# ChainBreak/denoising_diffusion_deep_fake

Hardware: AMD Instinct MI355X
Metric: training images/sec (256x256 U-Net, bs=16/GPU) (higher is better)
Workload: dtype f32; 1 GPU; d3f train_denoiser step: noise blend -> Unet(resnet34) fwd -> (MSE+1-SSIM)/2 -> bwd -> Adam, 256x256 synthetic face crops, bs=16/GPU, random-init weights, train-mode BatchNorm; image_size=256, batch_per_gpu=16, global_batch=16, parallelism=dp1, graph_step=False, adam_overlap_tail=False, adam_overlap_tail_steps=0, ranks_seen=1, csrc_digest=830583e7fcebca8c

## Files before the change

### denoising_diffusion_deep_fake_amd/csrc/batchnorm.hip

```cpp
#include "common.h"
#include "pointwise.h"
#include "vec16.h"

#include <algorithm>
#include <type_traits>

namespace d3f {

constexpr float BN_EPS = 1e-5f, BN_MOMENTUM = 0.1f;

constexpr int BNF_SC = 32;
constexpr int BNF_MAX_ROWS = 1024;
#ifndef BNF_FWD_U_F32
#define BNF_FWD_U_F32 4
#endif
#ifndef BNF_BWD_U
#define BNF_BWD_U 2
#endif

__device__ __forceinline__ float2 bn_fwd_coef(double s1, double s2, double count, int c, const float* __restrict__ gamma,
                                              const float* __restrict__ beta, float eps, float momentum, bool store,
                                              float* __restrict__ running_mean, float* __restrict__ running_var,
                                              float* __restrict__ mean_o, float* __restrict__ invstd_o,
                                              float* __restrict__ scale_o, float* __restrict__ shift_o) {
  const double mean = s1 / count;
  double var = s2 / count - mean * mean;
  if (var < 0.0) var = 0.0;
  const double invstd = 1.0 / sqrt(var + (double)eps);
  const float g = gamma[c], bt = beta[c];
  const float sc = (float)((double)g * invstd), sf = (float)((double)bt - mean * (double)g * invstd);
  if (store) {
    mean_o[c] = (float)mean; invstd_o[c] = (float)invstd; scale_o[c] = sc; shift_o[c] = sf;
    if (running_mean != nullptr) {
      const double unbiased = count > 1.0 ? var * count / (count - 1.0) : var;
      running_mean[c] = (float)((1.0 - (double)momentum) * (double)running_mean[c] + (double)momentum * mean);
      running_var[c] = (float)((1.0 - (double)momentum) * (double)running_var[c] + (double)momentum * unbiased);
    }
  }
  return make_float2(sc, sf);
}

__device__ __forceinline__ float3 bn_bwd_coef(double s1, double s2, double count, int c, int C,
                                              const float* __restrict__ gamma, const float* __restrict__ invstd, bool store,
                                              float* __restrict__ dgamma, float* __restrict__ dbeta, float* __restrict__ k) {
  const float k0 = gamma[c] * invstd[c], k1 = (float)(s1 / count), k2 = (float)(s2 / count);
  if (store) {
    if (dgamma != nullptr) { dgamma[c] = (float)s2; dbeta[c] = (float)s1; }
    k[c] = k0; k[C + c] = k1; k[2 * C + c] = k2;
  }
  return make_float3(k0, k1, k2);
}

template <typename F> static void by_dtype(int dtype, F&& f) {
  if (dtype == D3F_F32) f((float*)nullptr);
  else f((bf16_t*)nullptr);
}

__device__ __forceinline__ void block_sum2(double& s1, double& s2) {
  __shared__ double red[2][4];
#pragma unroll
  for (int o = 32; o > 0; o >>= 1) {
    s1 += __shfl_xor(s1, o);
    s2 += __shfl_xor(s2, o);
  }
  if ((threadIdx.x & 63) == 0) {
    red[0][threadIdx.x >> 6] = s1;
    red[1][threadIdx.x >> 6] = s2;
  }
  __syncthreads();
  s1 = (red[0][0] + red[0][1]) + (red[0][2] + red[0][3]);
  s2 = (red[1][0] + red[1][1]) + (red[1][2] + red[1][3]);
}

__global__ __launch_bounds__(256) void bn_finalize_kernel(
    const float* __restrict__ stats, int tiles, int C, int Cpad, double count,
    const float* __restrict__ gamma, const float* __restrict__ beta, float eps, float momentum,
    float* __restrict__ running_mean, float* __restrict__ running_var, float* __restrict__ mean_o,
    float* __restrict__ invstd_o, float* __restrict__ scale_o, float* __restrict__ shift_o, NetSplit ns) {
  chain_priority();
  if (blockIdx.z != 0) {
    net_shift(stats, ns.ws); net_shift(gamma, ns.par); net_shift(beta, ns.par);
    net_shift(running_mean, ns.bn); net_shift(running_var, ns.bn);
    net_shift(mean_o, ns.ws); net_shift(invstd_o, ns.ws); net_shift(scale_o, ns.ws); net_shift(shift_o, ns.ws);
  }
  const int c = blockIdx.x;
  double s1 = 0.0, s2 = 0.0;
  for (int t = threadIdx.x; t < tiles; t += 256) {
    const float2 v = *reinterpret_cast<const float2*>(stats + ((long)t * Cpad + c) * 2);
    s1 += (double)v.x;
    s2 += (double)v.y;
  }
  block_sum2(s1, s2);
  if (threadIdx.x == 0)
    bn_fwd_coef(s1, s2, count, c, gamma, beta, eps, momentum, true, running_mean, running_var, mean_o, invstd_o, scale_o,
                shift_o);
}

__global__ __launch_bounds__(256) void bn_eval_coeff_all_kernel(const float* __restrict__ params,
                                                                const float* __restrict__ bnstats,
                                                                char* __restrict__ ws, float eps, BnEvalTable t) {
  const BnEvalEntry e = t.e[blockIdx.x];
  float* __restrict__ coef = reinterpret_cast<float*>(ws + (size_t)e.coef_off16 * 16);
  for (int c = threadIdx.x; c < e.C; c += 256) {
    const float invstd = 1.0f / sqrtf(bnstats[e.rv_off + c] + eps);
    const float sc = params[e.g_off + c] * invstd;
    coef[2 * e.C + c] = sc;
    coef[3 * e.C + c] = params[e.b_off + c] - bnstats[e.rm_off + c] * sc;
  }
}

static_assert(BN_SCALE == 2 && BN_SHIFT == 3, "bn_eval_coeff_all_kernel writes the scale / shift rows");
int bn_eval_coeff_all_launch(const float* params, const float* bnstats, void* ws, const BnEvalTable& t,
                             hipStream_t stream) {
  if (t.n == 0) return 0;
  hipLaunchKernelGGL(bn_eval_coeff_all_kernel, dim3(t.n), dim3(256), 0, stream, params, bnstats, (char*)ws, BN_EPS, t);
  D3F_HIP(hipGetLastError());
  return 0;
}

template <typename T>
__global__ __launch_bounds__(256) void bn_apply_kernel(
    const T* __restrict__ y, const float* __restrict__ scale, const float* __restrict__ shift,
    const T* __restrict__ res, const T* __restrict__ yr, const float* __restrict__ scale_r,
    const float* __restrict__ shift_r, int relu, T* __restrict__ out, long nvec, int C, long net_ws) {
  chain_priority();
  if (blockIdx.z != 0) {
    net_shift(y, net_ws); net_shift(scale, net_ws); net_shift(shift, net_ws); net_shift(res, net_ws); net_shift(yr, net_ws);
    net_shift(scale_r, net_ws); net_shift(shift_r, net_ws); net_shift(out, net_ws);
  }
  constexpr int N = V16<T>::N;
  for (long i = (long)blockIdx.x * 256 + threadIdx.x; i < nvec; i += (long)gridDim.x * 256) {
    const int c0 = (int)((i * N) % C);
    float v[N], sc[N], sf[N];
    V16<T>::load(y + i * N, v);
#pragma unroll
    for (int k = 0; k < N; k += 4) {
      const float4 a = *reinterpret_cast<const float4*>(scale + c0 + k);
      const float4 b = *reinterpret_cast<const float4*>(shift + c0 + k);
      sc[k] = a.x; sc[k + 1] = a.y; sc[k + 2] = a.z; sc[k + 3] = a.w;
      sf[k] = b.x; sf[k + 1] = b.y; sf[k + 2] = b.z; sf[k + 3] = b.w;
    }
#pragma unroll
    for (int k = 0; k < N; ++k) v[k] = v[k] * sc[k] + sf[k];
    if (res != nullptr) {
      float r[N];
      V16<T>::load(res + i * N, r);
#pragma unroll
      for (int k = 0; k < N; ++k) v[k] += r[k];
    } else if (yr != nullptr) {
      float r[N];
      V16<T>::load(yr + i * N, r);
#pragma unroll
      for (int k = 0; k < N; ++k) v[k] += r[k] * scale_r[c0 + k] + shift_r[c0 + k];
    }
    if (relu) {
#pragma unroll
      for (int k = 0; k < N; ++k) v[k] = fmaxf(v[k], 0.f);
    }
    V16<T>::store(out + i * N, v);
  }
}



template <typename T>
__global__ __launch_bounds__(256) void bn_bwd_reduce_kernel(
    const T* __restrict__ dA, const T* __restrict__ a, const T* __restrict__ y,
    const float* __restrict__ mean, const float* __restrict__ invstd, float* __restrict__ partial,
    long rows, int C, const float* __restrict__ mask_scale, const float* __restrict__ mask_shift, long net_ws) {
  chain_priority();
  if (blockIdx.z != 0) {
    net_shift(dA, net_ws); net_shift(a, net_ws); net_shift(y, net_ws); net_shift(mean, net_ws); net_shift(invstd, net_ws);
    net_shift(partial, net_ws); net_shift(mask_scale, net_ws); net_shift(mask_shift, net_ws);
  }
  constexpr int N = V16<T>::N;
  __shared__ float red[256 * N * 2];
  const int VC = C / N;
  const int RP = 256 / VC;
  const int cv = threadIdx.x % VC, r0 = threadIdx.x / VC;
  const long rows_per_block = (rows + gridDim.x - 1) / gridDim.x;
  const long rbeg = (long)blockIdx.x * rows_per_block;
  long rend = rbeg + rows_per_block;
  if (rend > rows) rend = rows;
  float mu[N], is[N], s1[N], s2[N], msc[N], msf[N];
#pragma unroll
  for (int k = 0; k < N; ++k) {
    mu[k] = mean[cv * N + k];
    is[k] = invstd[cv * N + k];
    msc[k] = mask_scale ? mask_scale[cv * N + k] : 0.f;
    msf[k] = mask_scale ? mask_shift[cv * N + k] : 0.f;
    s1[k] = 0.f;
    s2[k] = 0.f;
  }
  constexpr int U = 4;
  const bool from_y = mask_scale != nullptr, from_a = !from_y && a != nullptr;
  long r = rbeg + r0;
  for (; r + (U - 1) * RP < rend; r += U * RP) {
    float g[U][N], yy[U][N], aa[U][N];
#pragma unroll
    for (int u = 0; u < U; ++u) {
      const long off = (r + u * RP) * C + cv * N;
      V16<T>::load(dA + off, g[u]);
      V16<T>::load(y + off, yy[u]);
      if (from_a) V16<T>::load(a + off, aa[u]);
    }
#pragma unroll
    for (int u = 0; u < U; ++u) {
#pragma unroll
      for (int k = 0; k < N; ++k) {
        const float keep = from_y ? yy[u][k] * msc[k] + msf[k] : (from_a ? aa[u][k] : 1.f);
        const float gz = keep > 0.f ? g[u][k] : 0.f;
        s1[k] += gz;
        s2[k] += gz * ((yy[u][k] - mu[k]) * is[k]);
      }
    }
  }
  for (; r < rend; r += RP) {
    const long off = r * C + cv * N;
    float g[N], yy[N], aa[N];
    V16<T>::load(dA + off, g);
    V16<T>::load(y + off, yy);
    if (from_a) V16<T>::load(a + off, aa);
#pragma unroll
    for (int k = 0; k < N; ++k) {
      const float keep = from_y ? yy[k] * msc[k] + msf[k] : (from_a ? aa[k] : 1.f);
      const float gz = keep > 0.f ? g[k] : 0.f;
      s1[k] += gz;
      s2[k] += gz * ((yy[k] - mu[k]) * is[k]);
    }
  }
#pragma unroll
  for (int k = 0; k < N; ++k) {
    red[(threadIdx.x * N + k) * 2 + 0] = s1[k];
    red[(threadIdx.x * N + k) * 2 + 1] = s2[k];
  }
  __syncthreads();
  for (int t = threadIdx.x; t < 2 * C; t += 256) {
    const int c = t >> 1, which = t & 1;
    const int v = c / N, k = c % N;
    float s = 0.f;
    for (int rr = 0; rr < RP; ++rr) s += red[((rr * VC + v) * N + k) * 2 + which];
    partial[((long)blockIdx.x * C + c) * 2 + which] = s;
  }
}

__global__ __launch_bounds__(256) void bn_bwd_finalize_kernel(
    const float* __restrict__ partial, int nblocks, int C, double count,
    const float* __restrict__ gamma, const float* __restrict__ invstd, float* __restrict__ dgamma,
    float* __restrict__ dbeta, float* __restrict__ coef, NetSplit ns) {
  chain_priority();
  if (blockIdx.z != 0) {
    net_shift(partial, ns.ws); net_shift(gamma, ns.par); net_shift(invstd, ns.ws);
    net_shift(dgamma, ns.grad); net_shift(dbeta, ns.grad); net_shift(coef, ns.ws);
  }
  const int c = blockIdx.x;
  double s1 = 0.0, s2 = 0.0;
  for (int t = threadIdx.x; t < nblocks; t += 256) {
    const float2 v = *reinterpret_cast<const float2*>(partial + ((long)t * C + c) * 2);
    s1 += (double)v.x;
    s2 += (double)v.y;
  }
  block_sum2(s1, s2);
  if (threadIdx.x == 0) bn_bwd_coef(s1, s2, count, c, C, gamma, invstd, true, dgamma, dbeta, coef);
}

template <typename T>
__global__ __launch_bounds__(256) void bn_bwd_apply_kernel(
    const T* __restrict__ dA, const T* __restrict__ a, const T* __restrict__ y,
    const float* __restrict__ mean, const float* __restrict__ invstd, const float* __restrict__ coef,
    T* __restrict__ dy, T* __restrict__ dres, int dres_acc, long nvec, int C,
    const float* __restrict__ mask_scale, const float* __restrict__ mask_shift, long net_ws) {
  chain_priority();
  if (blockIdx.z != 0) {
    net_shift(dA, net_ws); net_shift(a, net_ws); net_shift(y, net_ws); net_shift(mean, net_ws); net_shift(invstd, net_ws);
    net_shift(coef, net_ws); net_shift(dy, net_ws); net_shift(dres, net_ws); net_shift(mask_scale, net_ws);
    net_shift(mask_shift, net_ws);
  }
  constexpr int N = V16<T>::N;
  for (long i = (long)blockIdx.x * 256 + threadIdx.x; i < nvec; i += (long)gridDim.x * 256) {
    const int c0 = (int)((i * N) % C);
    float g[N], yy[N], o[N];
    V16<T>::load(dA + i * N, g);
    V16<T>::load(y + i * N, yy);
    if (mask_scale != nullptr) {
#pragma unroll
      for (int k = 0; k < N; ++k) g[k] = (yy[k] * mask_scale[c0 + k] + mask_shift[c0 + k]) > 0.f ? g[k] : 0.f;
    } else if (a != nullptr) {
      float aa[N];
      V16<T>::load(a + i * N, aa);
#pragma unroll
      for (int k = 0; k < N; ++k) g[k] = aa[k] > 0.f ? g[k] : 0.f;
    }
#pragma unroll
    for (int k = 0; k < N; ++k) {
      const int c = c0 + k;
      const float xhat = (yy[k] - mean[c]) * invstd[c];
      o[k] = coef[c] * (g[k] - coef[C + c] - xhat * coef[2 * C + c]);
    }
    V16<T>::store(dy + i * N, o);
    if (dres != nullptr) {
      if (dres_acc) {
        float d[N];
        V16<T>::load(dres + i * N, d);
#pragma unroll
        for (int k = 0; k < N; ++k) g[k] += d[k];
      }
      V16<T>::store(dres + i * N, g);
    }
  }
}

template <typename T> struct Raw4;
template <> struct Raw4<float> { typedef float4 type; };
template <> struct Raw4<bf16_t> { typedef uint2 type; };
__device__ __forceinline__ float4 ldraw(const float* p) { return *reinterpret_cast<const float4*>(p); }
__device__ __forceinline__ uint2 ldraw(const bf16_t* p) { return *reinterpret_cast<const uint2*>(p); }
__device__ __forceinline__ float4 cvt4(const float4& v) { return v; }
__device__ __forceinline__ float4 cvt4(const uint2& v) {
  return make_float4(__uint_as_float(v.x << 16), __uint_as_float(v.x & 0xffff0000u), __uint_as_float(v.y << 16),
                     __uint_as_float(v.y & 0xffff0000u));
}

template <typename F>
__device__ __forceinline__ void slab_reduce(const float* __restrict__ partial, int rows, int ld, int c0,
                                            double (&red)[16][64], double (&tot)[64], F behind_first_loads) {
  const int tid = threadIdx.x, q = tid & 15, rl = tid >> 4;
  double a0 = 0.0, a1 = 0.0, a2 = 0.0, a3 = 0.0;
  const float* base = partial + ((long)c0 * 2 + q * 4);
  int r = rl;
  bool hooked = false;
  for (; r + 112 < rows; r += 128) {
    float4 v[8];
#pragma unroll
    for (int j = 0; j < 8; ++j) v[j] = *reinterpret_cast<const float4*>(base + (long)(r + 16 * j) * ld * 2);
    if (!hooked) { behind_first_loads(); hooked = true; }
#pragma unroll
    for (int j = 0; j < 8; ++j) {
      a0 += (double)v[j].x; a1 += (double)v[j].y; a2 += (double)v[j].z; a3 += (double)v[j].w;
    }
  }
  for (; r + 48 < rows; r += 64) {
    const float4 v0 = *reinterpret_cast<const float4*>(base + (long)r * ld * 2);
    const float4 v1 = *reinterpret_cast<const float4*>(base + (long)(r + 16) * ld * 2);
    const float4 v2 = *reinterpret_cast<const float4*>(base + (long)(r + 32) * ld * 2);
    const float4 v3 = *reinterpret_cast<const float4*>(base + (long)(r + 48) * ld * 2);
    if (!hooked) { behind_first_loads(); hooked = true; }
    a0 += (double)v0.x; a1 += (double)v0.y; a2 += (double)v0.z; a3 += (double)v0.w;
    a0 += (double)v1.x; a1 += (double)v1.y; a2 += (double)v1.z; a3 += (double)v1.w;
    a0 += (double)v2.x; a1 += (double)v2.y; a2 += (double)v2.z; a3 += (double)v2.w;
    a0 += (double)v3.x; a1 += (double)v3.y; a2 += (double)v3.z; a3 += (double)v3.w;
  }
  if (!hooked) behind_first_loads();
  for (; r < rows; r += 16) {
    const float4 v = *reinterpret_cast<const float4*>(base + (long)r * ld * 2);
    a0 += (double)v.x; a1 += (double)v.y; a2 += (double)v.z; a3 += (double)v.w;
  }
  red[rl][q * 4 + 0] = a0;
  red[rl][q * 4 + 1] = a1;
  red[rl][q * 4 + 2] = a2;
  red[rl][q * 4 + 3] = a3;
  __syncthreads();
  if (tid < 64) {
    double s = 0.0;
#pragma unroll
    for (int k = 0; k < 16; ++k) s += red[k][tid];
    tot[tid] = s;
  }
  __syncthreads();
}

template <typename T, bool HAS2>
__global__ __launch_bounds__(256) void bn_finalize_apply_kernel(
    const float* __restrict__ stats, int stat_rows, int C, int Cpad, double count,
    const float* __restrict__ gamma, const float* __restrict__ beta, float eps, float momentum,
    float* __restrict__ running_mean, float* __restrict__ running_var, float* __restrict__ mean_o,
    float* __restrict__ invstd_o, float* __restrict__ scale_o, float* __restrict__ shift_o,
    const T* __restrict__ y, const T* __restrict__ res, const T* __restrict__ yr,
    const float* __restrict__ scale_r, const float* __restrict__ shift_r, int relu, T* __restrict__ out,
    long rows, long rows_per_block, NetSplit ns) {
  chain_priority();
  if (blockIdx.z != 0) {
    net_shift(stats, ns.ws); net_shift(gamma, ns.par); net_shift(beta, ns.par);
    net_shift(running_mean, ns.bn); net_shift(running_var, ns.bn);
    net_shift(mean_o, ns.ws); net_shift(invstd_o, ns.ws); net_shift(scale_o, ns.ws); net_shift(shift_o, ns.ws);
    net_shift(y, ns.ws); net_shift(res, ns.ws); net_shift(yr, ns.ws); net_shift(scale_r, ns.ws); net_shift(shift_r, ns.ws);
    net_shift(out, ns.ws);
  }
  __shared__ double red[16][64];
  __shared__ double tot[64];
  __shared__ float cf[2][BNF_SC];
  typedef typename Raw4<T>::type raw_t;
  constexpr int U = sizeof(T) == 4 ? BNF_FWD_U_F32 : 8;
  const int tid = threadIdx.x, c0 = blockIdx.y * BNF_SC;
  const int v = tid & 7, rr = tid >> 3, cc = c0 + v * 4;
  const long r0 = (long)blockIdx.x * rows_per_block;
  long r1 = r0 + rows_per_block;
  if (r1 > rows) r1 = rows;
  const T* __restrict__ second = res != nullptr ? res : yr;
  raw_t a[U], b[U], an[U], bn[U];
  auto load = [&](raw_t (&ya)[U], raw_t (&yb)[U], long r) {
#pragma unroll
    for (int u = 0; u < U; ++u) {
      const long row = r + 32 * u < r1 ? r + 32 * u : r1 - 1;
      ya[u] = ldraw(y + row * C + cc);
      if (HAS2) yb[u] = ldraw(second + row * C + cc);
    }
  };
  slab_reduce(stats, stat_rows, Cpad, c0, red, tot, [&]() { load(a, b, r0 + rr); });
  if (tid < BNF_SC) {
    const float2 f = bn_fwd_coef(tot[2 * tid], tot[2 * tid + 1], count, c0 + tid, gamma, beta, eps, momentum,
                                 blockIdx.x == 0, running_mean, running_var, mean_o, invstd_o, scale_o, shift_o);
    cf[0][tid] = f.x;
    cf[1][tid] = f.y;
  }
  __syncthreads();
  float sc[4], sf[4], scr[4] = {0.f, 0.f, 0.f, 0.f}, sfr[4] = {0.f, 0.f, 0.f, 0.f};
#pragma unroll
  for (int k = 0; k < 4; ++k) {
    sc[k] = cf[0][v * 4 + k];
    sf[k] = cf[1][v * 4 + k];
    if (HAS2 && res == nullptr) {
      scr[k] = scale_r[cc + k];
      sfr[k] = shift_r[cc + k];
    }
  }
  for (long r = r0 + rr; r < r1; r += 32 * U) {
    if (r + 32 * U < r1) load(an, bn, r + 32 * U);
#pragma unroll
    for (int u = 0; u < U; ++u) {
      const long row = r + 32 * u;
      if (row >= r1) continue;
      const float4 ya = cvt4(a[u]);
      float x[4] = {ya.x, ya.y, ya.z, ya.w};
#pragma unroll
      for (int k = 0; k < 4; ++k) x[k] = x[k] * sc[k] + sf[k];
      if (HAS2) {
        const float4 yb = cvt4(b[u]);
        if (res != nullptr) {
          x[0] += yb.x; x[1] += yb.y; x[2] += yb.z; x[3] += yb.w;
        } else {
          const float t[4] = {yb.x, yb.y, yb.z, yb.w};
#pragma unroll
          for (int k = 0; k < 4; ++k) x[k] += t[k] * scr[k] + sfr[k];
        }
      }
      if (relu) {
#pragma unroll
        for (int k = 0; k < 4; ++k) x[k] = fmaxf(x[k], 0.f);
      }
      st4<T>(out + row * C + cc, make_float4(x[0], x[1], x[2], x[3]));
    }
#pragma unroll
    for (int u = 0; u < U; ++u) {
      a[u] = an[u];
      if (HAS2) b[u] = bn[u];
    }
  }
}

static long rows_per_block_for(long rows, int slabs, int dtype, int plan_nets) {
  const long wgs = (dtype == D3F_F32 ? 256 : 512) / plan_nets_for(plan_nets, 64);
  long rb = std::max(1L, wgs / slabs);
  long rpb = (rows + rb - 1) / rb;
  rpb = (rpb + 31) / 32 * 32;
  return std::max(32L, rpb);
}

struct BnResidualOps {
  const void *res = nullptr, *yr = nullptr;
  const float *scale_r = nullptr, *shift_r = nullptr;
};
static BnResidualOps residual_ops(const BnLayer& L, const BnBufs& b) {
  if (L.res == BN_RES_TENSOR) return {b.res, nullptr, nullptr, nullptr};
  if (L.res == BN_RES_LAYER) return {nullptr, b.res, bn_coef(b.res_coef, L.C, BN_SCALE), bn_coef(b.res_coef, L.C, BN_SHIFT)};
  return {};
}

static int bn_finalize_apply_launch(const BnLayer& L, const BnBufs& b, hipStream_t stream, const NetSplit* ns) {
  if (L.rows == 0) return 0;
  const NetSplit nv = net_split_or_single(ns);
  const dim3 grid((unsigned)((L.rows + L.rows_per_block - 1) / L.rows_per_block), (unsigned)(L.C / BNF_SC),
                  (unsigned)nv.nets);
  const BnResidualOps r = residual_ops(L, b);
  by_dtype(L.dtype, [&](auto* typed) {
    typedef std::remove_pointer_t<decltype(typed)> T;
    auto go = [&](auto kernel) {
      hipLaunchKernelGGL(kernel, grid, dim3(256), 0, stream, b.stats, L.fwd_rows, L.C, L.Cpad, (double)L.rows, b.gamma,
                         b.beta, BN_EPS, BN_MOMENTUM, b.running_mean, b.running_var, bn_coef(b.coef, L.C, BN_MEAN),
                         bn_coef(b.coef, L.C, BN_INVSTD), bn_coef(b.coef, L.C, BN_SCALE), bn_coef(b.coef, L.C, BN_SHIFT),
                         (const T*)b.y, (const T*)r.res, (const T*)r.yr, r.scale_r, r.shift_r, L.relu ? 1 : 0, (T*)b.a,
                         L.rows, L.rows_per_block, nv);
    };
    if (L.res != BN_RES_NONE) go(bn_finalize_apply_kernel<T, true>);
    else go(bn_finalize_apply_kernel<T, false>);
  });
  D3F_HIP(hipGetLastError());
  return 0;
}

template <typename T, bool FROM_A, bool RD_DRES>
__global__ __launch_bounds__(256) void bn_bwd_finalize_apply_kernel(
    const float* __restrict__ partial, int nblocks, int C, double count, const float* __restrict__ gamma,
    const float* __restrict__ mean, const float* __restrict__ invstd, float* __restrict__ dgamma,
    float* __restrict__ dbeta, float* __restrict__ coef, const T* __restrict__ dA,
    const T* __restrict__ a, const T* __restrict__ y, T* __restrict__ dy, T* __restrict__ dres,
    long rows, long rows_per_block, const float* __restrict__ mask_scale,
    const float* __restrict__ mask_shift, NetSplit ns) {
  chain_priority();
  if (blockIdx.z != 0) {
    net_shift(partial, ns.ws); net_shift(gamma, ns.par); net_shift(mean, ns.ws); net_shift(invstd, ns.ws);
    net_shift(dgamma, ns.grad); net_shift(dbeta, ns.grad); net_shift(coef, ns.ws);
    net_shift(dA, ns.ws); net_shift(a, ns.ws); net_shift(y, ns.ws); net_shift(dy, ns.ws); net_shift(dres, ns.ws);
    net_shift(mask_scale, ns.ws); net_shift(mask_shift, ns.ws);
  }
  __shared__ double red[16][64];
  __shared__ double tot[64];
  __shared__ float cf[3][BNF_SC];
  typedef typename Raw4<T>::type raw_t;
  constexpr int U = BNF_BWD_U;
  const int tid = threadIdx.x, c0 = blockIdx.y * BNF_SC;
  const int v = tid & 7, rr = tid >> 3, cc = c0 + v * 4;
  const long r0 = (long)blockIdx.x * rows_per_block;
  long r1 = r0 + rows_per_block;
  if (r1 > rows) r1 = rows;
  raw_t g4[U], y4[U], a4[U], d4[U], g4n[U], y4n[U], a4n[U], d4n[U];
  auto load = [&](raw_t (&gg)[U], raw_t (&yy)[U], raw_t (&aa)[U], raw_t (&dd)[U], long r) {
#pragma unroll
    for (int u = 0; u < U; ++u) {
      const long row = r + 32 * u < r1 ? r + 32 * u : r1 - 1;
      gg[u] = ldraw(dA + row * C + cc);
      yy[u] = ldraw(y + row * C + cc);
      if (FROM_A) aa[u] = ldraw(a + row * C + cc);
      if (RD_DRES) dd[u] = ldraw(dres + row * C + cc);
    }
  };
  slab_reduce(partial, nblocks, C, c0, red, tot, [&]() { load(g4, y4, a4, d4, r0 + rr); });
  if (tid < BNF_SC) {
    const float3 k = bn_bwd_coef(tot[2 * tid], tot[2 * tid + 1], count, c0 + tid, C, gamma, invstd, blockIdx.x == 0,
                                 dgamma, dbeta, coef);
    cf[0][tid] = k.x;
    cf[1][tid] = k.y;
    cf[2][tid] = k.z;
  }
  __syncthreads();
  float k0[4], k1[4], k2[4], mu[4], is[4], msc[4] = {0.f, 0.f, 0.f, 0.f}, msf[4] = {0.f, 0.f, 0.f, 0.f};
#pragma unroll
  for (int k = 0; k < 4; ++k) {
    k0[k] = cf[0][v * 4 + k];
    k1[k] = cf[1][v * 4 + k];
    k2[k] = cf[2][v * 4 + k];
    mu[k] = mean[cc + k];
    is[k] = invstd[cc + k];
    if (!FROM_A && mask_scale != nullptr) {
      msc[k] = mask_scale[cc + k];
      msf[k] = mask_shift[cc + k];
    }
  }
  for (long r = r0 + rr; r < r1; r += 32 * U) {
    if (r + 32 * U < r1) load(g4n, y4n, a4n, d4n, r + 32 * U);
#pragma unroll
    for (int u = 0; u < U; ++u) {
      const long row = r + 32 * u;
      if (row >= r1) continue;
      const float4 gv = cvt4(g4[u]), yv = cvt4(y4[u]);
      float g[4] = {gv.x, gv.y, gv.z, gv.w};
      const float yy[4] = {yv.x, yv.y, yv.z, yv.w};
      if (FROM_A) {
        const float4 av = cvt4(a4[u]);
        const float aa[4] = {av.x, av.y, av.z, av.w};
#pragma unroll
        for (int k = 0; k < 4; ++k) g[k] = aa[k] > 0.f ? g[k] : 0.f;
      } else if (mask_scale != nullptr) {
#pragma unroll
        for (int k = 0; k < 4; ++k) g[k] = (yy[k] * msc[k] + msf[k]) > 0.f ? g[k] : 0.f;
      }
      float o[4];
#pragma unroll
      for (int k = 0; k < 4; ++k) {
        const float xhat = (yy[k] - mu[k]) * is[k];
        o[k] = k0[k] * (g[k] - k1[k] - xhat * k2[k]);
      }
      st4<T>(dy + row * C + cc, make_float4(o[0], o[1], o[2], o[3]));
      if (dres != nullptr) {
        if (RD_DRES) {
          const float4 dv = cvt4(d4[u]);
          g[0] += dv.x; g[1] += dv.y; g[2] += dv.z; g[3] += dv.w;
        }
        st4<T>(dres + row * C + cc, make_float4(g[0], g[1], g[2], g[3]));
      }
    }
#pragma unroll
    for (int u = 0; u < U; ++u) {
      g4[u] = g4n[u];
      y4[u] = y4n[u];
      if (FROM_A) a4[u] = a4n[u];
      if (RD_DRES) d4[u] = d4n[u];
    }
  }
}

struct BnBwdOps {
  const float *mean, *invstd;
  float* k;
  const void* a;
  const float *mask_scale, *mask_shift;
};
static BnBwdOps bwd_ops(const BnLayer& L, const BnBufs& b) {
  const bool from_y = L.mask == BN_MASK_FROM_Y;
  return {bn_coef(b.coef, L.C, BN_MEAN), bn_coef(b.coef, L.C, BN_INVSTD), b.k != nullptr ? b.k : bn_coef(b.coef, L.C, BN_K),
          L.mask == BN_MASK_FROM_A ? b.a : nullptr, from_y ? bn_coef(b.coef, L.C, BN_SCALE) : nullptr,
          from_y ? bn_coef(b.coef, L.C, BN_SHIFT) : nullptr};
}

static int bn_bwd_finalize_apply_launch(const BnLayer& L, const BnBufs& b, const BnBwdOps& o, hipStream_t stream,
                                        const NetSplit* ns) {
  if (L.rows == 0) return 0;
  const NetSplit nv = net_split_or_single(ns);
  const dim3 grid((unsigned)((L.rows + L.rows_per_block - 1) / L.rows_per_block), (unsigned)(L.C / BNF_SC),
                  (unsigned)nv.nets);
  const bool from_a = o.mask_scale == nullptr && o.a != nullptr;
  const bool rd_dres = b.dres != nullptr && b.dres_acc;
  by_dtype(L.dtype, [&](auto* typed) {
    typedef std::remove_pointer_t<decltype(typed)> T;
    auto go = [&](auto kernel) {
      hipLaunchKernelGGL(kernel, grid, dim3(256), 0, stream, b.stats, L.bwd_rows, L.C, (double)L.rows, b.gamma, o.mean,
                         o.invstd, b.dgamma, b.dbeta, o.k, (const T*)b.dA, (const T*)o.a, (const T*)b.y, (T*)b.dy,
                         (T*)b.dres, L.rows, L.rows_per_block, o.mask_scale, o.mask_shift, nv);
    };
    if (from_a && rd_dres) go(bn_bwd_finalize_apply_kernel<T, true, true>);
    else if (from_a) go(bn_bwd_finalize_apply_kernel<T, true, false>);
    else if (rd_dres) go(bn_bwd_finalize_apply_kernel<T, false, true>);
    else go(bn_bwd_finalize_apply_kernel<T, false, false>);
  });
  D3F_HIP(hipGetLastError());
  return 0;
}

void bn_layer_plan(BnLayer& L) {
  static const bool no_fused = getenv("D3F_NO_BN_FUSED_FINALIZE") != nullptr;
  auto fused_ok = [&](int rows) {
    return L.allow_fused && !no_fused && (L.dtype == D3F_F32 || L.dtype == D3F_BF16) && L.C % BNF_SC == 0 && rows >= 1 &&
           rows <= BNF_MAX_ROWS;
  };
  const long min_rows = std::max(16L, 4L * (256 / std::max(1, std::min(256, L.C / (L.dtype == D3F_F32 ? 4 : 8)))));
  L.reduce_blocks = (int)std::clamp((L.rows + min_rows - 1) / min_rows, 1L, 1024L);
  L.bwd_rows = L.fused_rows > 0 ? L.fused_rows : L.reduce_blocks;
  L.fwd_fused = L.apply && fused_ok(L.fwd_rows);
  L.bwd_fused = fused_ok(L.bwd_rows);
  L.rows_per_block = L.fwd_fused || L.bwd_fused ? rows_per_block_for(L.rows, L.C / BNF_SC, L.dtype, L.plan_nets) : 0;
  L.stat_floats = (size_t)L.fwd_rows * L.Cpad * 2;
  L.part_floats = (size_t)std::max(L.reduce_blocks, L.fused_rows) * L.C * 2;
}

int bn_layer_finalize(const BnLayer& L, const BnBufs& b, long count, hipStream_t stream, const NetSplit* ns) {
  const NetSplit nv = net_split_or_single(ns);
  hipLaunchKernelGGL(bn_finalize_kernel, dim3(L.C, 1, nv.nets), dim3(256), 0, stream, b.stats, L.fwd_rows, L.C, L.Cpad,
                     (double)count, b.gamma, b.beta, BN_EPS, BN_MOMENTUM, b.running_mean, b.running_var,
                     bn_coef(b.coef, L.C, BN_MEAN), bn_coef(b.coef, L.C, BN_INVSTD), bn_coef(b.coef, L.C, BN_SCALE),
                     bn_coef(b.coef, L.C, BN_SHIFT), nv);
  D3F_HIP(hipGetLastError());
  return 0;
}

int bn_layer_apply(const BnLayer& L, const BnBufs& b, hipStream_t stream, const NetSplit* ns) {
  const int ve = L.dtype == D3F_F32 ? 4 : 8;
  D3F_CHECK(L.C % ve == 0 && (256 * ve) % L.C == 0, "bn_apply: C=%d must divide %d", L.C, 256 * ve);
  const long nvec = L.rows * L.C / ve;
  if (nvec == 0) return 0;
  const NetSplit nv = net_split_or_single(ns);
  const BnResidualOps r = residual_ops(L, b);
  by_dtype(L.dtype, [&](auto* typed) {
    typedef std::remove_pointer_t<decltype(typed)> T;
    hipLaunchKernelGGL(bn_apply_kernel<T>, dim3(grid_for(nvec), 1, nv.nets), dim3(256), 0, stream, (const T*)b.y,
                       bn_coef(b.coef, L.C, BN_SCALE), bn_coef(b.coef, L.C, BN_SHIFT), (const T*)r.res, (const T*)r.yr,
                       r.scale_r, r.shift_r, L.relu ? 1 : 0, (T*)b.a, nvec, L.C, nv.ws);
  });
  D3F_HIP(hipGetLastError());
  return 0;
}

int bn_layer_forward(const BnLayer& L, const BnBufs& b, const BnSync* sync, hipStream_t stream, const NetSplit* ns) {
  long count = L.rows;
  if (sync != nullptr) {
    if (int rc = sync->fn(sync->ctx, b.stats, (int64_t)L.fwd_rows * L.Cpad * 2, (void*)stream))
      return set_error(rc, "BatchNorm statistics all-reduce failed in the forward pass (%s)", L.name.c_str());
    count *= sync->world;
  } else if (L.fwd_fused) {
    return bn_finalize_apply_launch(L, b, stream, ns);
  }
  if (int rc = bn_layer_finalize(L, b, count, stream, ns)) return rc;
  return L.apply ? bn_layer_apply(L, b, stream, ns) : 0;
}

int bn_layer_backward(const BnLayer& L, const BnBufs& b, const BnSync* sync, hipStream_t stream, const NetSplit* ns) {
  const int C = L.C, ve = L.dtype == D3F_F32 ? 4 : 8, vc = C / ve;
  const NetSplit nv = net_split_or_single(ns);
  const BnBwdOps o = bwd_ops(L, b);
  if (L.fused_rows == 0) {
    D3F_CHECK(C % ve == 0 && vc >= 1 && vc <= 256 && (256 % vc) == 0, "bn_bwd_reduce: unsupported channel count %d", C);
    by_dtype(L.dtype, [&](auto* typed) {
      typedef std::remove_pointer_t<decltype(typed)> T;
      hipLaunchKernelGGL(bn_bwd_reduce_kernel<T>, dim3(L.reduce_blocks, 1, nv.nets), dim3(256), 0, stream,
                         (const T*)b.dA, (const T*)o.a, (const T*)b.y, o.mean, o.invstd, b.stats, L.rows, C, o.mask_scale,
                         o.mask_shift, nv.ws);
    });
    D3F_HIP(hipGetLastError());
  }
  auto finalize = [&](long count, float* dgamma, float* dbeta) -> int {
    hipLaunchKernelGGL(bn_bwd_finalize_kernel, dim3(C, 1, nv.nets), dim3(256), 0, stream, b.stats, L.bwd_rows, C,
                       (double)count, b.gamma, o.invstd, dgamma, dbeta, o.k, nv);
    D3F_HIP(hipGetLastError());
    return 0;
  };
  if (sync != nullptr) {
    if (int rc = finalize(L.rows, b.dgamma, b.dbeta)) return rc;
    if (int rc = sync->fn(sync->ctx, b.stats, (int64_t)L.bwd_rows * C * 2, (void*)stream))
      return set_error(rc, "BatchNorm statistics all-reduce failed in the backward pass (%s)", L.name.c_str());
    if (int rc = finalize(L.rows * sync->world, nullptr, nullptr)) return rc;
  } else if (L.bwd_fused) {
    return bn_bwd_finalize_apply_launch(L, b, o, stream, ns);
  } else if (int rc = finalize(L.rows, b.dgamma, b.dbeta)) {
    return rc;
  }
  D3F_CHECK(C % ve == 0 && (256 * ve) % C == 0, "bn_bwd_apply: C=%d must divide %d", C, 256 * ve);
  const long nvec = L.rows * C / ve;
  if (nvec == 0) return 0;
  by_dtype(L.dtype, [&](auto* typed) {
    typedef std::remove_pointer_t<decltype(typed)> T;
    hipLaunchKernelGGL(bn_bwd_apply_kernel<T>, dim3(grid_for(nvec), 1, nv.nets), dim3(256), 0, stream, (const T*)b.dA,
                       (const T*)o.a, (const T*)b.y, o.mean, o.invstd, o.k, (T*)b.dy, (T*)b.dres, b.dres_acc, nvec, C,
                       o.mask_scale, o.mask_shift, nv.ws);
  });
  D3F_HIP(hipGetLastError());
  return 0;
}

}
```

### denoising_diffusion_deep_fake_amd/csrc/loss.hip

```cpp
#include "pointwise.h"
#include "philox.h"

namespace d3f {

constexpr int SS_T = 32;
constexpr int SS_K = 11;
constexpr int SS_IN = SS_T + SS_K - 1;
constexpr int SS_LD = SS_IN + 1;

struct GaussK {
  float g[SS_K];
};

static GaussK make_gauss() {
  GaussK k;
  float s = 0.f;
  for (int i = 0; i < SS_K; ++i) {
    const float d = (float)i - (float)(SS_K - 1) / 2.f;
    k.g[i] = expf(-(d * d) / (2.f * 1.5f * 1.5f));
    s += k.g[i];
  }
  for (int i = 0; i < SS_K; ++i) k.g[i] /= s;
  return k;
}

__device__ __forceinline__ float norm01(float v, float lo, float range) {
  const float t = (v - lo) / range;
  return fminf(fmaxf(t, 0.f), 1.f);
}

__global__ __launch_bounds__(256) void ssim_fwd_kernel(const float* __restrict__ pred,
                                                       const float* __restrict__ target, float lo,
                                                       float range, GaussK gk, int H, int W,
                                                       float* __restrict__ dA, float* __restrict__ dB,
                                                       float* __restrict__ dC,
                                                       float* __restrict__ partial) {
  chain_priority();
  __shared__ float tx[SS_IN * SS_LD], ty[SS_IN * SS_LD];
  __shared__ float vv[5][SS_T * SS_LD];
  __shared__ float wsum[4];
  const int Hv = H - (SS_K - 1), Wv = W - (SS_K - 1);
  const int plane = blockIdx.z;
  const int oy0 = blockIdx.y * SS_T, ox0 = blockIdx.x * SS_T;
  const float* __restrict__ px = pred + (long)plane * H * W;
  const float* __restrict__ py = target + (long)plane * H * W;
  const int tid = threadIdx.x;
  for (int e = tid; e < SS_IN * SS_IN; e += 256) {
    const int r = e / SS_IN, c = e - r * SS_IN;
    const int iy = oy0 + r, ix = ox0 + c;
    float a = 0.f, b = 0.f;
    if (iy < H && ix < W) {
      a = norm01(px[(long)iy * W + ix], lo, range);
      b = norm01(py[(long)iy * W + ix], lo, range);
    }
    tx[r * SS_LD + c] = a;
    ty[r * SS_LD + c] = b;
  }
  __syncthreads();
  constexpr int RB = 8;
  if (tid < SS_IN * (SS_T / RB)) {
    const int c = tid % SS_IN, r0 = (tid / SS_IN) * RB;
    float a[RB + SS_K - 1], b[RB + SS_K - 1], aa[RB + SS_K - 1], bb[RB + SS_K - 1], ab[RB + SS_K - 1];
#pragma unroll
    for (int i = 0; i < RB + SS_K - 1; ++i) {
      a[i] = tx[(r0 + i) * SS_LD + c];
      b[i] = ty[(r0 + i) * SS_LD + c];
      aa[i] = a[i] * a[i];
      bb[i] = b[i] * b[i];
      ab[i] = a[i] * b[i];
    }
#pragma unroll
    for (int r = 0; r < RB; ++r) {
      float s0 = 0.f, s1 = 0.f, s2 = 0.f, s3 = 0.f, s4 = 0.f;
#pragma unroll
      for (int i = 0; i < SS_K; ++i) {
        const float g = gk.g[i];
        s0 += g * a[r + i];
        s1 += g * b[r + i];
        s2 += g * aa[r + i];
        s3 += g * bb[r + i];
        s4 += g * ab[r + i];
      }
      vv[0][(r0 + r) * SS_LD + c] = s0;
      vv[1][(r0 + r) * SS_LD + c] = s1;
      vv[2][(r0 + r) * SS_LD + c] = s2;
      vv[3][(r0 + r) * SS_LD + c] = s3;
      vv[4][(r0 + r) * SS_LD + c] = s4;
    }
  }
  __syncthreads();
  const float c1 = 0.01f * 0.01f, c2 = 0.03f * 0.03f;
  float local = 0.f;
  constexpr int CBk = 4;
  const int rr = tid / (SS_T / CBk), cq = (tid % (SS_T / CBk)) * CBk;
  float win[5][CBk + SS_K - 1];
#pragma unroll
  for (int q = 0; q < 5; ++q)
#pragma unroll
    for (int j = 0; j < CBk + SS_K - 1; ++j) win[q][j] = vv[q][rr * SS_LD + cq + j];
#pragma unroll
  for (int cc = 0; cc < CBk; ++cc) {
    const int r = rr, c = cq + cc;
    const int oy = oy0 + r, ox = ox0 + c;
    if (oy >= Hv || ox >= Wv) continue;
    float m[5];
#pragma unroll
    for (int q = 0; q < 5; ++q) {
      float s = 0.f;
#pragma unroll
      for (int j = 0; j < SS_K; ++j) s += gk.g[j] * win[q][cc + j];
      m[q] = s;
    }
    const float mux = m[0], muy = m[1];
    const float sxx = m[2] - mux * mux, syy = m[3] - muy * muy, sxy = m[4] - mux * muy;
    const float a1 = 2.f * mux * muy + c1, b1 = mux * mux + muy * muy + c1;
    const float a2 = 2.f * sxy + c2, b2 = sxx + syy + c2;
    const float l = a1 / b1, cs = a2 / b2;
    const float ss = l * cs;
    local += ss;
    const long o = ((long)plane * Hv + oy) * Wv + ox;
    const float dl_dmux = 2.f * (muy - l * mux) / b1;
    const float dcs_dmux = (2.f * mux * cs - 2.f * muy) / b2;
    dA[o] = cs * dl_dmux + l * dcs_dmux;
    dB[o] = -l * cs / b2;
    dC[o] = 2.f * l / b2;
  }
#pragma unroll
  for (int o = 32; o > 0; o >>= 1) local += __shfl_xor(local, o);
  if ((tid & 63) == 0) wsum[tid >> 6] = local;
  __syncthreads();
  if (tid == 0)
    partial[((long)blockIdx.z * gridDim.y + blockIdx.y) * gridDim.x + blockIdx.x] =
        (wsum[0] + wsum[1]) + (wsum[2] + wsum[3]);
}

__global__ __launch_bounds__(256) void ssim_mse_bwd_kernel(
    const float* __restrict__ pred, const float* __restrict__ target, float lo, float range, GaussK gk,
    int H, int W, const float* __restrict__ dA, const float* __restrict__ dB,
    const float* __restrict__ dC, float ssim_coef, float mse_coef, float* __restrict__ grad,
    float* __restrict__ partial_mse) {
  chain_priority();
  __shared__ float t3[3][SS_IN * SS_LD];
  __shared__ float vv[3][SS_T * SS_LD];
  __shared__ float wsum[4];
  const int Hv = H - (SS_K - 1), Wv = W - (SS_K - 1);
  const int plane = blockIdx.z;
  const int py0 = blockIdx.y * SS_T, px0 = blockIdx.x * SS_T;
  const int tid = threadIdx.x;
  for (int e = tid; e < SS_IN * SS_IN; e += 256) {
    const int r = e / SS_IN, c = e - r * SS_IN;
    const int oy = py0 - (SS_K - 1) + r, ox = px0 - (SS_K - 1) + c;
    float a = 0.f, b = 0.f, d = 0.f;
    if (oy >= 0 && oy < Hv && ox >= 0 && ox < Wv) {
      const long o = ((long)plane * Hv + oy) * Wv + ox;
      a = dA[o];
      b = dB[o];
      d = dC[o];
    }
    t3[0][r * SS_LD + c] = a;
    t3[1][r * SS_LD + c] = b;
    t3[2][r * SS_LD + c] = d;
  }
  __syncthreads();
  constexpr int RB = 8;
  if (tid < SS_IN * (SS_T / RB)) {
    const int c = tid % SS_IN, r0 = (tid / SS_IN) * RB;
    float v0[RB + SS_K - 1], v1[RB + SS_K - 1], v2[RB + SS_K - 1];
#pragma unroll
    for (int i = 0; i < RB + SS_K - 1; ++i) {
      v0[i] = t3[0][(r0 + i) * SS_LD + c];
      v1[i] = t3[1][(r0 + i) * SS_LD + c];
      v2[i] = t3[2][(r0 + i) * SS_LD + c];
    }
#pragma unroll
    for (int r = 0; r < RB; ++r) {
      float s0 = 0.f, s1 = 0.f, s2 = 0.f;
#pragma unroll
      for (int i = 0; i < SS_K; ++i) {
        const float g = gk.g[SS_K - 1 - i];
        s0 += g * v0[r + i];
        s1 += g * v1[r + i];
        s2 += g * v2[r + i];
      }
      vv[0][(r0 + r) * SS_LD + c] = s0;
      vv[1][(r0 + r) * SS_LD + c] = s1;
      vv[2][(r0 + r) * SS_LD + c] = s2;
    }
  }
  __syncthreads();
  const float inv_range = 1.f / range;
  float local = 0.f;
  constexpr int CBk = 4;
  const int rr = tid / (SS_T / CBk), cq = (tid % (SS_T / CBk)) * CBk;
  float win[3][CBk + SS_K - 1];
#pragma unroll
  for (int q = 0; q < 3; ++q)
#pragma unroll
    for (int j = 0; j < CBk + SS_K - 1; ++j) win[q][j] = vv[q][rr * SS_LD + cq + j];
#pragma unroll
  for (int cc = 0; cc < CBk; ++cc) {
    const int r = rr, c = cq + cc;
    const int iy = py0 + r, ix = px0 + c;
    if (iy >= H || ix >= W) continue;
    float ga = 0.f, gb = 0.f, gc = 0.f;
#pragma unroll
    for (int j = 0; j < SS_K; ++j) {
      const float g = gk.g[SS_K - 1 - j];
      ga += g * win[0][cc + j];
      gb += g * win[1][cc + j];
      gc += g * win[2][cc + j];
    }
    const long p = (long)plane * H * W + (long)iy * W + ix;
    const float pv = pred[p], tv = target[p];
    const float rawx = (pv - lo) / range;
    const float xh = fminf(fmaxf(rawx, 0.f), 1.f);
    const float yh = norm01(tv, lo, range);
    float gx = ga + 2.f * xh * gb + yh * gc;
    gx = (rawx >= 0.f && rawx <= 1.f) ? gx * inv_range : 0.f;
    const float diff = pv - tv;
    local += diff * diff;
    grad[p] = ssim_coef * gx + mse_coef * diff;
  }
#pragma unroll
  for (int o = 32; o > 0; o >>= 1) local += __shfl_xor(local, o);
  if ((tid & 63) == 0) wsum[tid >> 6] = local;
  __syncthreads();
  if (tid == 0)
    partial_mse[((long)blockIdx.z * gridDim.y + blockIdx.y) * gridDim.x + blockIdx.x] =
        (wsum[0] + wsum[1]) + (wsum[2] + wsum[3]);
}

__global__ __launch_bounds__(256) void loss_finalize_kernel(const float* __restrict__ part_ss, int n_ss,
                                                            const float* __restrict__ part_mse,
                                                            int n_mse, double n_ssim_elems,
                                                            double n_elems, float* __restrict__ out) {
  chain_priority();
  __shared__ double red[2][256];
  double a = 0.0, b = 0.0;
  for (int i = threadIdx.x; i < n_ss; i += 256) a += (double)part_ss[i];
  for (int i = threadIdx.x; i < n_mse; i += 256) b += (double)part_mse[i];
  red[0][threadIdx.x] = a;
  red[1][threadIdx.x] = b;
  __syncthreads();
  for (int s = 128; s > 0; s >>= 1) {
    if (threadIdx.x < s) {
      red[0][threadIdx.x] += red[0][threadIdx.x + s];
      red[1][threadIdx.x] += red[1][threadIdx.x + s];
    }
    __syncthreads();
  }
  if (threadIdx.x == 0) {
    const float ssim = (float)(red[0][0] / n_ssim_elems);
    const float mse = (float)(red[1][0] / n_elems);
    out[0] = (mse + (1.0f - ssim)) / 2.0f;
    out[1] = mse;
    out[2] = ssim;
  }
}

static inline int tiles(int n) { return (n + SS_T - 1) / SS_T; }

size_t loss_workspace_floats(int B, int H, int W) {
  if (H < SS_K || W < SS_K) return 0;
  const long planes = (long)B * 3;
  const long maps = 3 * planes * (H - SS_K + 1) * (W - SS_K + 1);
  const long p1 = planes * tiles(H - SS_K + 1) * tiles(W - SS_K + 1);
  const long p2 = planes * tiles(H) * tiles(W);
  return (size_t)(maps + p1 + p2 + 16);
}

int mse_ssim_loss_launch(const float* pred, const float* target, float in_min, float in_max,
                         float* loss_out, float* grad_pred, float* workspace, int B, int H, int W,
                         hipStream_t stream) {
  D3F_CHECK(H >= SS_K && W >= SS_K, "loss: image %dx%d smaller than the 11x11 SSIM window", H, W);
  D3F_CHECK(in_max > in_min, "loss: input range");
  static const GaussK gk = make_gauss();
  const int Hv = H - SS_K + 1, Wv = W - SS_K + 1;
  const long planes = (long)B * 3;
  const long map = planes * Hv * Wv;
  float* dA = workspace;
  float* dB = dA + map;
  float* dC = dB + map;
  float* part_ss = dC + map;
  const int n_ss = (int)(planes * tiles(Hv) * tiles(Wv));
  float* part_mse = part_ss + n_ss;
  const int n_mse = (int)(planes * tiles(H) * tiles(W));
  const float range = in_max - in_min;
  hipLaunchKernelGGL(ssim_fwd_kernel, dim3(tiles(Wv), tiles(Hv), (unsigned)planes), dim3(256), 0, stream,
                     pred, target, in_min, range, gk, H, W, dA, dB, dC, part_ss);
  D3F_HIP(hipGetLastError());
  const double n_elems = (double)planes * H * W;
  const double n_ssim = (double)planes * Hv * Wv;
  const float ssim_coef = (float)(-0.5 / n_ssim);
  const float mse_coef = (float)(1.0 / n_elems);
  hipLaunchKernelGGL(ssim_mse_bwd_kernel, dim3(tiles(W), tiles(H), (unsigned)planes), dim3(256), 0,
                     stream, pred, target, in_min, range, gk, H, W, dA, dB, dC, ssim_coef, mse_coef,
                     grad_pred, part_mse);
  D3F_HIP(hipGetLastError());
  hipLaunchKernelGGL(loss_finalize_kernel, dim3(1), dim3(256), 0, stream, part_ss, n_ss, part_mse, n_mse,
                     n_ssim, n_elems, loss_out);
  D3F_HIP(hipGetLastError());
  return 0;
}

struct BlendCoef {
  float r, sa, sb;
};
__device__ __forceinline__ BlendCoef blend_coef(float y, float c, float one_minus_c, float inv_lam) {
  const float t = __fadd_rn(__fmul_rn(y, one_minus_c), c);
  const float r = inv_lam > 0.f ? __fmul_rn(inv_lam, (float)log((double)__fdiv_rn(1.0f, t))) : y;
  return BlendCoef{r, __fsqrt_rn(__fsub_rn(1.0f, r)), __fsqrt_rn(r)};
}
__device__ __forceinline__ float4 blend4(const BlendCoef k, const float4 a, const float4 n) {
  float4 o;
  o.x = __fadd_rn(__fmul_rn(k.sa, a.x), __fmul_rn(k.sb, n.x));
  o.y = __fadd_rn(__fmul_rn(k.sa, a.y), __fmul_rn(k.sb, n.y));
  o.z = __fadd_rn(__fmul_rn(k.sa, a.z), __fmul_rn(k.sb, n.z));
  o.w = __fadd_rn(__fmul_rn(k.sa, a.w), __fmul_rn(k.sb, n.w));
  return o;
}

__global__ __launch_bounds__(256) void noise_blend_kernel(const float* __restrict__ x,
                                                          const float* __restrict__ noise,
                                                          const float* __restrict__ y_uniform,
                                                          float c, float one_minus_c, float inv_lam,
                                                          float* __restrict__ out,
                                                          float* __restrict__ r_out, long per_image) {
  const int b = blockIdx.y;
  const BlendCoef k = blend_coef(y_uniform[b], c, one_minus_c, inv_lam);
  if (r_out != nullptr && blockIdx.x == 0 && threadIdx.x == 0) r_out[b] = k.r;
  const long nvec = per_image / 4;
  const float4* __restrict__ xv = reinterpret_cast<const float4*>(x + (long)b * per_image);
  const float4* __restrict__ nv = reinterpret_cast<const float4*>(noise + (long)b * per_image);
  float4* __restrict__ ov = reinterpret_cast<float4*>(out + (long)b * per_image);
  for (long i = (long)blockIdx.x * 256 + threadIdx.x; i < nvec; i += (long)gridDim.x * 256) ov[i] = blend4(k, xv[i], nv[i]);
}

int noise_blend_launch(const float* x, const float* noise, const float* y_uniform, float lam,
                       float* out, float* r_out, int B, long per_image, hipStream_t stream) {
  D3F_CHECK(per_image % 4 == 0, "noise_blend: per-image element count %ld not a multiple of 4", per_image);
  D3F_CHECK(lam > 0.f, "noise_blend: lambda must be positive");
  if (B == 0 || per_image == 0) return 0;
  const double c = 1.0 / exp((double)lam);
  long bx = (per_image / 4 + 255) / 256;
  if (bx > 256) bx = 256;
  hipLaunchKernelGGL(noise_blend_kernel, dim3((unsigned)bx, (unsigned)B), dim3(256), 0, stream, x, noise,
                     y_uniform, (float)c, (float)(1.0 - c), (float)(1.0 / (double)lam), out, r_out,
                     per_image);
  D3F_HIP(hipGetLastError());
  return 0;
}

int noise_blend_fixed_launch(const float* x, const float* noise, const float* r, float* out, int B, long per_image,
                             hipStream_t stream) {
  D3F_CHECK(per_image % 4 == 0, "noise_blend: per-image element count %ld not a multiple of 4", per_image);
  if (B == 0 || per_image == 0) return 0;
  long bx = (per_image / 4 + 255) / 256;
  if (bx > 256) bx = 256;
  hipLaunchKernelGGL(noise_blend_kernel, dim3((unsigned)bx, (unsigned)B), dim3(256), 0, stream, x, noise, r, 0.f, 0.f,
                     -1.f, out, (float*)nullptr, per_image);
  D3F_HIP(hipGetLastError());
  return 0;
}

__global__ __launch_bounds__(256) void noise_blend_rng_kernel(const float* __restrict__ x, uint64_t seed, uint64_t offset,
                                                              const float* __restrict__ y_or_r, float c,
                                                              float one_minus_c, float inv_lam, float* __restrict__ out,
                                                              float* __restrict__ r_out, long per_image) {
  chain_priority();
  const int b = blockIdx.y;
  const BlendCoef k = blend_coef(y_or_r != nullptr ? y_or_r[b] : rng_y(seed, offset, b), c, one_minus_c, inv_lam);
  if (r_out != nullptr && blockIdx.x == 0 && threadIdx.x == 0) r_out[b] = k.r;
  const long nvec = per_image / 4;
  const float4* __restrict__ xv = reinterpret_cast<const float4*>(x + (long)b * per_image);
  float4* __restrict__ ov = reinterpret_cast<float4*>(out + (long)b * per_image);
  for (long i = (long)blockIdx.x * 256 + threadIdx.x; i < nvec; i += (long)gridDim.x * 256)
    ov[i] = blend4(k, xv[i], rng_normal4(seed, offset, b, (uint32_t)i));
}

__global__ __launch_bounds__(256) void noise_draw_kernel(uint64_t seed, uint64_t offset, float* __restrict__ noise,
                                                         float* __restrict__ y, long per_image) {
  const int b = blockIdx.y;
  if (y != nullptr && blockIdx.x == 0 && threadIdx.x == 0) y[b] = rng_y(seed, offset, b);
  if (noise == nullptr) return;
  const long nvec = per_image / 4;
  float4* __restrict__ nv = reinterpret_cast<float4*>(noise + (long)b * per_image);
  for (long i = (long)blockIdx.x * 256 + threadIdx.x; i < nvec; i += (long)gridDim.x * 256)
    nv[i] = rng_normal4(seed, offset, b, (uint32_t)i);
}

static int rng_shape_check(const char* what, long per_image) {
  D3F_CHECK(per_image % 4 == 0, "%s: per-image element count %ld not a multiple of 4", what, per_image);
  D3F_CHECK(per_image / 4 < (long)RNG_G_APPLY, "%s: per-image element count %ld leaves no room for the reserved groups",
            what, per_image);
  return 0;
}
static unsigned rng_blocks(long per_image) {
  const long bx = (per_image / 4 + 255) / 256;
  return (unsigned)(bx > 256 ? 256 : (bx < 1 ? 1 : bx));
}

int noise_blend_rng_launch(const float* x, uint64_t seed, uint64_t offset, float lam, float* out, float* r_out, int B,
                           long per_image, hipStream_t stream) {
  if (int rc = rng_shape_check("noise_blend_rng", per_image)) return rc;
  D3F_CHECK(lam > 0.f, "noise_blend_rng: lambda must be positive");
  if (B == 0 || per_image == 0) return 0;
  const double c = 1.0 / exp((double)lam);
  hipLaunchKernelGGL(noise_blend_rng_kernel, dim3(rng_blocks(per_image), (unsigned)B), dim3(256), 0, stream, x, seed,
                     offset, (const float*)nullptr, (float)c, (float)(1.0 - c), (float)(1.0 / (double)lam), out, r_out,
                     per_image);
  D3F_HIP(hipGetLastError());
  return 0;
}

int noise_blend_fixed_rng_launch(const float* x, uint64_t seed, uint64_t offset, const float* r, float* out, int B,
                                 long per_image, hipStream_t stream) {
  if (int rc = rng_shape_check("noise_blend_fixed_rng", per_image)) return rc;
  if (B == 0 || per_image == 0) return 0;
  hipLaunchKernelGGL(noise_blend_rng_kernel, dim3(rng_blocks(per_image), (unsigned)B), dim3(256), 0, stream, x, seed,
                     offset, r, 0.f, 0.f, -1.f, out, (float*)nullptr, per_image);
  D3F_HIP(hipGetLastError());
  return 0;
}

int noise_draw_launch(uint64_t seed, uint64_t offset, float* noise, float* y, int B, long per_image,
                      hipStream_t stream) {
  if (int rc = rng_shape_check("noise_draw", per_image)) return rc;
  if (B == 0 || (noise == nullptr && y == nullptr)) return 0;
  const unsigned bx = (noise != nullptr && per_image > 0) ? rng_blocks(per_image) : 1u;
  hipLaunchKernelGGL(noise_draw_kernel, dim3(bx, (unsigned)B), dim3(256), 0, stream, seed, offset,
                     per_image > 0 ? noise : (float*)nullptr, y, per_image);
  D3F_HIP(hipGetLastError());
  return 0;
}

__global__ __launch_bounds__(256) void l1_partial_kernel(const float* __restrict__ p, const float* __restrict__ t,
                                                         double* __restrict__ partial, long per_image) {
  __shared__ double red[256];
  const int b = blockIdx.y;
  const float* pp = p + (long)b * per_image;
  const float* tt = t + (long)b * per_image;
  double s = 0.0;
  for (long i = (long)blockIdx.x * 256 + threadIdx.x; i < per_image; i += (long)gridDim.x * 256)
    s += (double)fabsf(pp[i] - tt[i]);
  red[threadIdx.x] = s;
  __syncthreads();
  for (int o = 128; o > 0; o >>= 1) {
    if ((int)threadIdx.x < o) red[threadIdx.x] += red[threadIdx.x + o];
    __syncthreads();
  }
  if (threadIdx.x == 0) partial[(long)b * L1_PARTS + blockIdx.x] = red[0];
}
__global__ void l1_finalize_kernel(const double* __restrict__ partial, float* __restrict__ out, int B, long per_image) {
  const int b = blockIdx.x * blockDim.x + threadIdx.x;
  if (b >= B) return;
  out[b] = l1_image_mean(partial, b, per_image);
}
size_t l1_per_image_workspace_bytes(int B) { return (size_t)B * L1_PARTS * sizeof(double) + 64; }
int l1_partials_launch(const float* pred, const float* target, double* partial, int B, long per_image,
                       hipStream_t stream) {
  hipLaunchKernelGGL(l1_partial_kernel, dim3(L1_PARTS, (unsigned)B), dim3(256), 0, stream, pred, target, partial,
                     per_image);
  D3F_HIP(hipGetLastError());
  return 0;
}
int l1_per_image_launch(const float* pred, const float* target, float* out, void* workspace, int B, long per_image,
                        hipStream_t stream) {
  if (B == 0) return 0;
  double* partial = reinterpret_cast<double*>(workspace);
  if (int rc = l1_partials_launch(pred, target, partial, B, per_image, stream)) return rc;
  hipLaunchKernelGGL(l1_finalize_kernel, dim3((B + 63) / 64), dim3(64), 0, stream, partial, out, B, per_image);
  D3F_HIP(hipGetLastError());
  return 0;
}

}
```

### denoising_diffusion_deep_fake_amd/csrc/pointwise.hip

```cpp
#include "pointwise.h"
#include "philox.h"
#include "vec16.h"

namespace d3f {

template <typename T>
__global__ __launch_bounds__(256) void maxpool_fwd_kernel(const T* __restrict__ in, T* __restrict__ out,
                                                          uint8_t* __restrict__ idx, int B, int H,
                                                          int W, int C, long net_ws) {
  chain_priority();
  if (blockIdx.z != 0) {
    net_shift(in, net_ws); net_shift(out, net_ws); net_shift(idx, net_ws);
  }
  constexpr int N = V16<T>::N;
  const int Ho = H / 2, Wo = W / 2, VC = C / N;
  const long total = (long)B * Ho * Wo * VC;
  for (long i = (long)blockIdx.x * 256 + threadIdx.x; i < total; i += (long)gridDim.x * 256) {
    const int cv = (int)(i % VC);
    long t = i / VC;
    const int ox = (int)(t % Wo);
    t /= Wo;
    const int oy = (int)(t % Ho);
    const int b = (int)(t / Ho);
    float best[N];
    int bi[N];
    bool first = true;
#pragma unroll
    for (int kh = 0; kh < 3; ++kh) {
      const int iy = 2 * oy - 1 + kh;
      if ((unsigned)iy >= (unsigned)H) continue;
#pragma unroll
      for (int kw = 0; kw < 3; ++kw) {
        const int ix = 2 * ox - 1 + kw;
        if ((unsigned)ix >= (unsigned)W) continue;
        float v[N];
        V16<T>::load(in + (((long)b * H + iy) * W + ix) * C + cv * N, v);
        if (first) {
#pragma unroll
          for (int k = 0; k < N; ++k) { best[k] = v[k]; bi[k] = kh * 3 + kw; }
          first = false;
        } else {
#pragma unroll
          for (int k = 0; k < N; ++k)
            if (v[k] > best[k] || v[k] != v[k]) { best[k] = v[k]; bi[k] = kh * 3 + kw; }
        }
      }
    }
    const long o = (((long)b * Ho + oy) * Wo + ox) * C + cv * N;
    V16<T>::store(out + o, best);
#pragma unroll
    for (int k = 0; k < N; ++k) idx[o + k] = (uint8_t)bi[k];
  }
}

template <typename T>
__global__ __launch_bounds__(256) void maxpool_bwd_kernel(const T* __restrict__ dout,
                                                          const uint8_t* __restrict__ idx,
                                                          T* __restrict__ din, int accumulate, int B,
                                                          int H, int W, int C, unsigned vc_mul, unsigned vc_shr,
                                                          long net_ws) {
  chain_priority();
  if (blockIdx.z != 0) {
    net_shift(dout, net_ws); net_shift(idx, net_ws); net_shift(din, net_ws);
  }
  constexpr int N = V16<T>::N;
  const int Ho = H / 2, Wo = W / 2, VC = C / N;
  const int j = (int)blockIdx.x * 256 + (int)threadIdx.x;
  if (j >= W * VC) return;
  const int ix = fast_div(j, vc_mul, vc_shr), cv = j - ix * VC;
  const int row = (int)blockIdx.y;
  const int iy = row % H, b = row / H;
  const int noy = (iy & 1) ? 2 : 1, nox = (ix & 1) ? 2 : 1;
  const int oy0 = (iy + 1) >> 1, kh0 = (iy & 1) ? 0 : 1;
  const int ox0 = (ix + 1) >> 1, kw0 = (ix & 1) ? 0 : 1;
  float g[N];
#pragma unroll
  for (int k = 0; k < N; ++k) g[k] = 0.f;
#pragma unroll
  for (int a = 0; a < 2; ++a) {
    const int oy = oy0 - a, kh = a ? 2 : kh0;
    if (a >= noy || oy >= Ho) continue;
#pragma unroll
    for (int c = 0; c < 2; ++c) {
      const int ox = ox0 - c, kw = c ? 2 : kw0;
      if (c < nox && ox < Wo) {
        const long o = (((long)b * Ho + oy) * Wo + ox) * C + cv * N;
        float d[N];
        V16<T>::load(dout + o, d);
        const unsigned tap = (unsigned)(kh * 3 + kw);
        uint32_t w[N / 4];
        if constexpr (N == 4) {
          w[0] = *reinterpret_cast<const uint32_t*>(idx + o);
        } else {
          const uint2 t = *reinterpret_cast<const uint2*>(idx + o);
          w[0] = t.x;
          w[1] = t.y;
        }
#pragma unroll
        for (int k = 0; k < N; ++k)
          if (((w[k >> 2] >> (8 * (k & 3))) & 0xffu) == tap) g[k] += d[k];
      }
    }
  }
  T* dst = din + ((long)row * W * VC + j) * N;
  if (accumulate) {
    float old[N];
    V16<T>::load(dst, old);
#pragma unroll
    for (int k = 0; k < N; ++k) g[k] += old[k];
  }
  V16<T>::store(dst, g);
}

int maxpool3x3s2_fwd_launch(int dtype, const void* in, void* out, uint8_t* idx, int B, int H, int W,
                            int C, hipStream_t stream, const NetSplit* ns) {
  const int ve = dtype == D3F_F32 ? 4 : 8;
  D3F_CHECK(C % ve == 0 && H % 2 == 0 && W % 2 == 0, "maxpool: shape (%d,%d,%d)", H, W, C);
  const long total = (long)B * (H / 2) * (W / 2) * (C / ve);
  if (total == 0) return 0;
  const NetSplit nv = net_split_or_single(ns);
  const dim3 grid(grid_for(total), 1, nv.nets);
  if (dtype == D3F_F32)
    hipLaunchKernelGGL(maxpool_fwd_kernel<float>, grid, dim3(256), 0, stream,
                       (const float*)in, (float*)out, idx, B, H, W, C, nv.ws);
  else
    hipLaunchKernelGGL(maxpool_fwd_kernel<bf16_t>, grid, dim3(256), 0, stream,
                       (const bf16_t*)in, (bf16_t*)out, idx, B, H, W, C, nv.ws);
  D3F_HIP(hipGetLastError());
  return 0;
}

int maxpool3x3s2_bwd_launch(int dtype, const void* dout, const uint8_t* idx, void* din, int accumulate,
                            int B, int H, int W, int C, hipStream_t stream, const NetSplit* ns) {
  const int ve = dtype == D3F_F32 ? 4 : 8;
  D3F_CHECK(C % ve == 0 && H % 2 == 0 && W % 2 == 0, "maxpool: shape (%d,%d,%d)", H, W, C);
  const NetSplit nv = net_split_or_single(ns);
  const long total = (long)B * H * W * (C / ve);
  if (total == 0) return 0;
  const int vc = C / ve;
  unsigned vc_mul, vc_shr;
  fast_div_setup((unsigned)vc, &vc_mul, &vc_shr);
  D3F_CHECK((long)B * H <= 65535, "maxpool backward: %d rows exceed the grid", B * H);
  const dim3 grid((unsigned)cdiv((long)W * vc, 256), (unsigned)(B * H), (unsigned)nv.nets);
  if (dtype == D3F_F32)
    hipLaunchKernelGGL(maxpool_bwd_kernel<float>, grid, dim3(256), 0, stream,
                       (const float*)dout, idx, (float*)din, accumulate, B, H, W, C, vc_mul, vc_shr, nv.ws);
  else
    hipLaunchKernelGGL(maxpool_bwd_kernel<bf16_t>, grid, dim3(256), 0, stream,
                       (const bf16_t*)dout, idx, (bf16_t*)din, accumulate, B, H, W, C, vc_mul, vc_shr, nv.ws);
  D3F_HIP(hipGetLastError());
  return 0;
}

template <typename T>
__global__ __launch_bounds__(256) void sum2x2_kernel(const T* __restrict__ dfull, T* __restrict__ dlow,
                                                     int B, int Hl, int Wl, int C, long net_ws) {
  chain_priority();
  if (blockIdx.z != 0) {
    net_shift(dfull, net_ws); net_shift(dlow, net_ws);
  }
  constexpr int N = V16<T>::N;
  const int VC = C / N;
  const long total = (long)B * Hl * Wl * VC;
  const int Wf = 2 * Wl;
  for (long i = (long)blockIdx.x * 256 + threadIdx.x; i < total; i += (long)gridDim.x * 256) {
    const int cv = (int)(i % VC);
    long t = i / VC;
    const int x = (int)(t % Wl);
    t /= Wl;
    const long base = ((t * 2) * Wf + 2 * x) * (long)C + cv * N;
    float s[N], v[N];
    V16<T>::load(dfull + base, s);
    V16<T>::load(dfull + base + C, v);
#pragma unroll
    for (int k = 0; k < N; ++k) s[k] += v[k];
    V16<T>::load(dfull + base + (long)Wf * C, v);
#pragma unroll
    for (int k = 0; k < N; ++k) s[k] += v[k];
    V16<T>::load(dfull + base + (long)Wf * C + C, v);
#pragma unroll
    for (int k = 0; k < N; ++k) s[k] += v[k];
    V16<T>::store(dlow + i * N, s);
  }
}

int sum2x2_launch(int dtype, const void* dfull, void* dlow, int B, int Hl, int Wl, int C,
                  hipStream_t stream, const NetSplit* ns) {
  const int ve = dtype == D3F_F32 ? 4 : 8;
  D3F_CHECK(C % ve == 0, "sum2x2: C=%d", C);
  const long total = (long)B * Hl * Wl * (C / ve);
  if (total == 0) return 0;
  const NetSplit nv = net_split_or_single(ns);
  const dim3 grid(grid_for(total), 1, nv.nets);
  if (dtype == D3F_F32)
    hipLaunchKernelGGL(sum2x2_kernel<float>, grid, dim3(256), 0, stream,
                       (const float*)dfull, (float*)dlow, B, Hl, Wl, C, nv.ws);
  else
    hipLaunchKernelGGL(sum2x2_kernel<bf16_t>, grid, dim3(256), 0, stream,
                       (const bf16_t*)dfull, (bf16_t*)dlow, B, Hl, Wl, C, nv.ws);
  D3F_HIP(hipGetLastError());
  return 0;
}

template <typename T>
__global__ __launch_bounds__(256) void nchw_to_nhwc_kernel(const float* __restrict__ in,
                                                           T* __restrict__ out, int B, int C, long HW,
                                                           int Cpad, long net_in, long net_ws) {
  if (blockIdx.z != 0) {
    net_shift(in, net_in); net_shift(out, net_ws);
  }
  const long total = (long)B * HW;
  for (long i = (long)blockIdx.x * 256 + threadIdx.x; i < total; i += (long)gridDim.x * 256) {
    const long b = i / HW, pix = i - b * HW;
    for (int c = 0; c < Cpad; ++c) {
      const float v = c < C ? in[(b * C + c) * HW + pix] : 0.f;
      out[i * Cpad + c] = from_f32<T>(v);
    }
  }
}

template <typename T>
__global__ __launch_bounds__(256) void nhwc_to_nchw_kernel(const T* __restrict__ in,
                                                           float* __restrict__ out, int B, int C,
                                                           long HW, int Cpad) {
  const long total = (long)B * HW;
  for (long i = (long)blockIdx.x * 256 + threadIdx.x; i < total; i += (long)gridDim.x * 256) {
    const long b = i / HW, pix = i - b * HW;
    for (int c = 0; c < C; ++c) out[(b * C + c) * HW + pix] = to_f32<T>(in[i * Cpad + c]);
  }
}

template <typename T>
__global__ __launch_bounds__(256) void u8bgr_to_nhwc_kernel(const uint8_t* __restrict__ in, T* __restrict__ out,
                                                            long npix, int Cpad, float m0, float m1, float m2,
                                                            float s0, float s1, float s2) {
  for (long i = (long)blockIdx.x * 256 + threadIdx.x; i < npix; i += (long)gridDim.x * 256) {
    const uint8_t* px = in + i * 3;
    const float r = ((float)px[2] - m0) / s0, g = ((float)px[1] - m1) / s1, b = ((float)px[0] - m2) / s2;
    T* o = out + i * Cpad;
    o[0] = from_f32<T>(r);
    o[1] = from_f32<T>(g);
    o[2] = from_f32<T>(b);
    for (int c = 3; c < Cpad; ++c) o[c] = from_f32<T>(0.f);
  }
}

__global__ __launch_bounds__(256) void nchw_to_u8bgr_kernel(const float* __restrict__ in, uint8_t* __restrict__ out,
                                                            int B, long HW, int W, long out_row_stride, float m0,
                                                            float m1, float m2, float s0, float s1, float s2) {
  const long total = (long)B * HW, H = HW / W;
  for (long i = (long)blockIdx.x * 256 + threadIdx.x; i < total; i += (long)gridDim.x * 256) {
    const long b = i / HW, pix = i - b * HW;
    const float* src = in + b * 3 * HW + pix;
    auto q = [](float y, float s, float m) {
      const float v = y * s + m;
      int t = (int)v;
      t = t < 0 ? 0 : (t > 255 ? 255 : t);
      return (uint8_t)t;
    };
    const long y = pix / W, x = pix - y * W;
    uint8_t* o = out + (b * H + y) * out_row_stride + x * 3;
    o[2] = q(src[0], s0, m0);
    o[1] = q(src[HW], s1, m1);
    o[0] = q(src[2 * HW], s2, m2);
  }
}

__global__ __launch_bounds__(256) void u8rgb_to_nchw_kernel(const uint8_t* __restrict__ in, float* __restrict__ out,
                                                            int B, long HW, U8Normalise norm) {
  const long total = (long)B * HW;
  for (long i = (long)blockIdx.x * 256 + threadIdx.x; i < total; i += (long)gridDim.x * 256) {
    const long b = i / HW, pix = i - b * HW;
    const uint8_t* px = in + i * 3;
    float* o = out + b * 3 * HW + pix;
    o[0] = norm(px[0], 0);
    o[HW] = norm(px[1], 1);
    o[2 * HW] = norm(px[2], 2);
  }
}

__global__ __launch_bounds__(256) void affine_warp_kernel(const float* __restrict__ in, const float* __restrict__ theta,
                                                          float* __restrict__ out, int B, int C, int H, int W) {
  const long HW = (long)H * W, total = (long)B * HW;
  for (long i = (long)blockIdx.x * 256 + threadIdx.x; i < total; i += (long)gridDim.x * 256) {
    const int b = (int)(i / HW);
    affine_warp_pixel(PlaneTexels{in + (long)b * C * HW, HW}, out + (long)b * C * HW, theta + b * 6,
                      (int)(i - (long)b * HW), C, H, W);
  }
}

int affine_warp_launch(const float* in, const float* theta, float* out, int B, int C, int H, int W,
                       hipStream_t stream) {
  const long total = (long)B * H * W;
  if (total == 0) return 0;
  hipLaunchKernelGGL(affine_warp_kernel, dim3(grid_for(total, 256, 8192)), dim3(256), 0, stream, in, theta, out, B, C,
                     H, W);
  D3F_HIP(hipGetLastError());
  return 0;
}

__global__ __launch_bounds__(256) void affine_warp_rng_kernel(const float* __restrict__ in, float* __restrict__ out,
                                                              uint64_t seed, uint64_t offset, AffineRngParams q, int C,
                                                              int H, int W) {
  __shared__ float th[6];
  __shared__ int warped;
  const int b = blockIdx.y;
  if (threadIdx.x == 0) {
    float t[6];
    warped = affine_theta_rng(seed, offset, b, q, t) ? 1 : 0;
    for (int k = 0; k < 6; ++k) th[k] = t[k];
  }
  __syncthreads();
  const long HW = (long)H * W;
  if (warped) {
    float t[6];
    for (int k = 0; k < 6; ++k) t[k] = th[k];
    const PlaneTexels src{in + (long)b * C * HW, HW};
    for (long pix = (long)blockIdx.x * 256 + threadIdx.x; pix < HW; pix += (long)gridDim.x * 256)
      affine_warp_pixel(src, out + (long)b * C * HW, t, (int)pix, C, H, W);
  } else {
    const long n = (long)C * HW;
    const float* __restrict__ src = in + (long)b * n;
    float* __restrict__ dst = out + (long)b * n;
    for (long i = (long)blockIdx.x * 256 + threadIdx.x; i < n; i += (long)gridDim.x * 256) dst[i] = src[i];
  }
}

__global__ __launch_bounds__(64) void affine_theta_draw_kernel(uint64_t seed, uint64_t offset, AffineRngParams q,
                                                               float* __restrict__ theta, uint8_t* __restrict__ apply,
                                                               int B) {
  const int b = blockIdx.x * 64 + threadIdx.x;
  if (b >= B) return;
  float t[6];
  const bool w = affine_theta_rng(seed, offset, b, q, t);
  if (theta != nullptr)
    for (int k = 0; k < 6; ++k) theta[(long)b * 6 + k] = t[k];
  if (apply != nullptr) apply[b] = w ? 1 : 0;
}

int affine_rng_params(int kind, const float params[5], int H, int W, AffineRngParams& q) {
  D3F_CHECK(kind == 0 || kind == 1, "affine rng: kind %d is neither 0 (RandomAffine) nor 1 (ShiftScaleRotate)", kind);
  D3F_CHECK(H > 0 && W > 0, "affine rng: bad shape");
  q = AffineRngParams{};
  q.kind = kind;
  q.deg2rad = (float)(M_PI / 180.0);
  q.h_over_w = (float)((double)H / (double)W);
  q.w_over_h = (float)((double)W / (double)H);
  if (kind == 0) {
    D3F_CHECK(params[3] > 0.f && params[4] >= params[3], "affine rng: scale range [%g, %g]", params[3], params[4]);
    q.angle_unit = (float)((double)params[0] * (M_PI / 180.0));
    q.shift_x = params[1], q.shift_y = params[2];
    q.scale_lo = params[3];
    q.scale_span = (float)((double)params[4] - (double)params[3]);
    q.p = 1.0f;
  } else {
    D3F_CHECK(params[1] >= 0.f && params[1] < 1.f, "affine rng: scale_limit %g outside [0, 1)", params[1]);
    q.shift_x = q.shift_y = params[0];
    q.scale_span = params[1];
    q.angle_unit = params[2];
    q.p = params[3];
  }
  return 0;
}

int affine_warp_rng_launch(const float* in, float* out, uint64_t seed, uint64_t offset, const AffineRngParams& q, int B,
                           int C, int H, int W, hipStream_t stream) {
  const long HW = (long)H * W;
  if ((long)B * HW == 0) return 0;
  D3F_CHECK((long)C * HW < (1L << 31), "affine_warp_rng: image of %ld elements", (long)C * HW);
  long bx = (HW + 255) / 256;
  if (bx > 128) bx = 128;
  hipLaunchKernelGGL(affine_warp_rng_kernel, dim3((unsigned)bx, (unsigned)B), dim3(256), 0, stream, in, out, seed, offset,
                     q, C, H, W);
  D3F_HIP(hipGetLastError());
  return 0;
}

int affine_theta_draw_launch(uint64_t seed, uint64_t offset, const AffineRngParams& q, float* theta, uint8_t* apply, int B,
                             hipStream_t stream) {
  if (B == 0) return 0;
  hipLaunchKernelGGL(affine_theta_draw_kernel, dim3((unsigned)((B + 63) / 64)), dim3(64), 0, stream, seed, offset, q,
                     theta, apply, B);
  D3F_HIP(hipGetLastError());
  return 0;
}

int u8bgr_to_nhwc_launch(int dtype, const uint8_t* in, void* out, long npix, int Cpad, const float mean255[3],
                         const float std255[3], hipStream_t stream) {
  if (npix == 0) return 0;
  if (dtype == D3F_F32)
    hipLaunchKernelGGL(u8bgr_to_nhwc_kernel<float>, dim3(grid_for(npix)), dim3(256), 0, stream, in, (float*)out, npix,
                       Cpad, mean255[0], mean255[1], mean255[2], std255[0], std255[1], std255[2]);
  else
    hipLaunchKernelGGL(u8bgr_to_nhwc_kernel<bf16_t>, dim3(grid_for(npix)), dim3(256), 0, stream, in, (bf16_t*)out,
                       npix, Cpad, mean255[0], mean255[1], mean255[2], std255[0], std255[1], std255[2]);
  D3F_HIP(hipGetLastError());
  return 0;
}

int u8rgb_to_nchw_launch(const uint8_t* in, float* out, int B, long HW, const float mean[3], const float stdv[3],
                         hipStream_t stream) {
  if ((long)B * HW == 0) return 0;
  hipLaunchKernelGGL(u8rgb_to_nchw_kernel, dim3(grid_for((long)B * HW)), dim3(256), 0, stream, in, out, B, HW,
                     U8Normalise{mean[0], mean[1], mean[2], stdv[0], stdv[1], stdv[2]});
  D3F_HIP(hipGetLastError());
  return 0;
}

int nchw_to_u8bgr_launch(const float* in, uint8_t* out, int B, int H, int W, long out_row_stride, const float mean255[3],
                         const float std255[3], hipStream_t stream) {
  const long HW = (long)H * W;
  if ((long)B * HW == 0) return 0;
  hipLaunchKernelGGL(nchw_to_u8bgr_kernel, dim3(grid_for((long)B * HW)), dim3(256), 0, stream, in, out, B, HW, W,
                     out_row_stride, mean255[0], mean255[1], mean255[2], std255[0], std255[1], std255[2]);
  D3F_HIP(hipGetLastError());
  return 0;
}

int nchw_to_nhwc_launch(int dtype, const float* in, void* out, int B, int C, int H, int W, int Cpad,
                        hipStream_t stream, const NetSplit* ns) {
  const long total = (long)B * H * W;
  if (total == 0) return 0;
  const NetSplit nv = net_split_or_single(ns);
  const dim3 grid(grid_for(total), 1, nv.nets);
  if (dtype == D3F_F32)
    hipLaunchKernelGGL(nchw_to_nhwc_kernel<float>, grid, dim3(256), 0, stream, in,
                       (float*)out, B, C, (long)H * W, Cpad, nv.in, nv.ws);
  else
    hipLaunchKernelGGL(nchw_to_nhwc_kernel<bf16_t>, grid, dim3(256), 0, stream, in,
                       (bf16_t*)out, B, C, (long)H * W, Cpad, nv.in, nv.ws);
  D3F_HIP(hipGetLastError());
  return 0;
}

int nhwc_to_nchw_launch(int dtype, const void* in, float* out, int B, int C, int H, int W, int Cpad,
                        hipStream_t stream) {
  const long total = (long)B * H * W;
  if (total == 0) return 0;
  if (dtype == D3F_F32)
    hipLaunchKernelGGL(nhwc_to_nchw_kernel<float>, dim3(grid_for(total)), dim3(256), 0, stream,
                       (const float*)in, out, B, C, (long)H * W, Cpad);
  else
    hipLaunchKernelGGL(nhwc_to_nchw_kernel<bf16_t>, dim3(grid_for(total)), dim3(256), 0, stream,
                       (const bf16_t*)in, out, B, C, (long)H * W, Cpad);
  D3F_HIP(hipGetLastError());
  return 0;
}

__device__ __forceinline__ int dgrad_tap_slot_to_flipped(int slot, int taps, int stride) {
  if (stride == 2 && taps == 9) return (int)((0x453718620ull >> (4 * slot)) & 15);
  return slot;
}
template <typename T, bool X3>
__device__ __forceinline__ void pack_store(T* __restrict__ base, long idx, long plane, float v) {
  if constexpr (X3) {
    const uint32_t xb = __float_as_uint(v), hb = xb & 0xffff0000u;
    const float r1 = v - __uint_as_float(hb);
    const uint32_t mb = __float_as_uint(r1) & 0xffff0000u;
    const float r2 = r1 - __uint_as_float(mb);
    base[idx] = (T)(hb >> 16);
    base[plane + idx] = (T)(mb >> 16);
    base[2 * plane + idx] = (T)(__float_as_uint(r2) >> 16);
  } else {
    base[idx] = from_f32<T>(v);
  }
}

__device__ __forceinline__ unsigned up_fwd_set(int parity, int a) {
  return parity == 0 ? (a == 0 ? 1u : 6u) : (a == 0 ? 3u : 4u);
}
__device__ __forceinline__ unsigned up_bwd_set(int u) { return u == 0 ? 4u : u == 1 ? 6u : u == 2 ? 3u : 1u; }

struct UpDiv {
  unsigned fplane[2], kc[2], c0[2], c1[2], k9[2], cd[2], k4[2];
};
template <typename T, bool X3>
__global__ __launch_bounds__(256) void pack_up_kernel(const float* __restrict__ w, int Cout, int C0, int C1,
                                                      T* __restrict__ wfc, int CoutPad, T* __restrict__ wd4,
                                                      int C0Rows, T* __restrict__ wds, int C1Rows, int CoutD,
                                                      int K9, UpDiv dv) {
  const int Cin = C0 + C1;
  const int Kc = 4 * C0 + 9 * C1, K4 = 16 * CoutD;
  const int nf = 4 * CoutPad * Kc, nd = C0Rows * K4, ns = C1Rows * K9;
  const int fplane = CoutPad * Kc;
  for (int i = (int)blockIdx.x * 256 + (int)threadIdx.x; i < nf + nd + ns; i += (int)gridDim.x * 256) {
    if (i < nf) {
      const int z = fast_div(i, dv.fplane[0], dv.fplane[1]);
      const int r = i - z * fplane;
      const int n = fast_div(r, dv.kc[0], dv.kc[1]), k = r - n * Kc;
      float v = 0.f;
      if (n < Cout) {
        if (k < 4 * C0) {
          const int ab = fast_div(k, dv.c0[0], dv.c0[1]), c = k - ab * C0;
          const unsigned sh = up_fwd_set(z >> 1, ab >> 1), sw = up_fwd_set(z & 1, ab & 1);
          const float* __restrict__ wp = w + ((long)n * Cin + c) * 9;
#pragma unroll
          for (int kh = 0; kh < 3; ++kh)
#pragma unroll
            for (int kw = 0; kw < 3; ++kw)
              if (((sh >> kh) & 1u) && ((sw >> kw) & 1u)) v += wp[kh * 3 + kw];
        } else {
          const int kk = k - 4 * C0, tap = fast_div(kk, dv.c1[0], dv.c1[1]), c1 = kk - tap * C1;
          v = w[((long)n * Cin + C0 + c1) * 9 + tap];
        }
      }
      pack_store<T, X3>(wfc + (X3 ? 3L * z * fplane : (long)z * fplane), r, fplane, v);
    } else if (i >= nf + nd) {
      const int j = i - nf - nd;
      const int c1 = fast_div(j, dv.k9[0], dv.k9[1]), k = j - c1 * K9;
      const int f = fast_div(k, dv.cd[0], dv.cd[1]), n = k - f * CoutD;
      float v = 0.f;
      if (c1 < C1 && n < Cout && f < 9) v = w[((long)n * Cin + C0 + c1) * 9 + (8 - f)];
      pack_store<T, X3>(wds, j, ns, v);
    } else {
      const int j = i - nf;
      const int c = fast_div(j, dv.k4[0], dv.k4[1]), k = j - c * K4;
      const int uv = fast_div(k, dv.cd[0], dv.cd[1]), n = k - uv * CoutD;
      float v = 0.f;
      if (c < C0 && n < Cout) {
        const unsigned sh = up_bwd_set(uv >> 2), sw = up_bwd_set(uv & 3);
        const float* __restrict__ wp = w + ((long)n * Cin + c) * 9;
#pragma unroll
        for (int kh = 0; kh < 3; ++kh)
#pragma unroll
          for (int kw = 0; kw < 3; ++kw)
            if (((sh >> kh) & 1u) && ((sw >> kw) & 1u)) v += wp[kh * 3 + kw];
      }
      pack_store<T, X3>(wd4, j, nd, v);
    }
  }
}

int pack_up_launch(int dtype, const float* w, int Cout, int C0, int C1, void* wfc, int CoutPad, void* wd4,
                   int C0Rows, void* wds, int C1Rows, hipStream_t stream) {
  const int ve = dtype == D3F_BF16 ? 8 : 4;
  const int CoutD = (int)round_up(Cout, ve);
  if (wd4 == nullptr) C0Rows = 0;
  if (wds == nullptr) C1Rows = 0;
  const int K9 = (int)round_up(9L * CoutD, dtype == D3F_BF16 ? 64 : 32);
  const long total = 4L * CoutPad * (4 * C0 + 9 * C1) + (long)C0Rows * 16 * CoutD + (long)C1Rows * K9;
  if (total == 0) return 0;
  D3F_CHECK(total < (1L << 31) - 2048L * 256, "pack_up: %ld elements exceed the 32-bit element index", total);
  UpDiv dv;
  auto setup = [](long d, unsigned (&o)[2]) { fast_div_setup((unsigned)(d > 0 ? d : 1), &o[0], &o[1]); };
  setup((long)CoutPad * (4 * C0 + 9 * C1), dv.fplane);
  setup(4 * C0 + 9 * C1, dv.kc);
  setup(C0, dv.c0);
  setup(C1, dv.c1);
  setup(K9, dv.k9);
  setup(CoutD, dv.cd);
  setup(16 * CoutD, dv.k4);
  if (dtype == D3F_F32)
    hipLaunchKernelGGL((pack_up_kernel<float, false>), dim3(grid_for(total)), dim3(256), 0, stream, w, Cout, C0, C1,
                       (float*)wfc, CoutPad, (float*)wd4, C0Rows, (float*)wds, C1Rows, CoutD, K9, dv);
  else if (dtype == D3F_F32X3)
    hipLaunchKernelGGL((pack_up_kernel<bf16_t, true>), dim3(grid_for(total)), dim3(256), 0, stream, w, Cout, C0, C1,
                       (bf16_t*)wfc, CoutPad, (bf16_t*)wd4, C0Rows, (bf16_t*)wds, C1Rows, CoutD, K9, dv);
  else
    hipLaunchKernelGGL((pack_up_kernel<bf16_t, false>), dim3(grid_for(total)), dim3(256), 0, stream, w, Cout, C0, C1,
                       (bf16_t*)wfc, CoutPad, (bf16_t*)wd4, C0Rows, (bf16_t*)wds, C1Rows, CoutD, K9, dv);
  D3F_HIP(hipGetLastError());
  return 0;
}

template <typename T, bool X3>
__global__ __launch_bounds__(256) void pack_all_kernel(const float* __restrict__ params, char* __restrict__ ws,
                                                       PackTable t) {
  __shared__ float tile[PACK_NT * (PACK_LDS_ROW + 1)];
  int l = 0;
  while (l + 1 < t.n && blockIdx.x >= t.e[l + 1].block0) ++l;
  const PackEntry e = t.e[l];
  const float* __restrict__ w = params + e.w_off;
  T* __restrict__ wf = reinterpret_cast<T*>(ws + (size_t)e.wf_off16 * 16);
  T* __restrict__ wd = reinterpret_cast<T*>(ws + (size_t)e.wd_off16 * 16);
  const int taps = e.taps, Cin = e.Cin, CinReal = e.CinReal, Cout = e.Cout, Kpad = e.Kpad, KpadD = e.KpadD,
            CoutD = e.CoutD, CT = e.CT, CoutPad = e.CoutPad, CinRows = e.CinRows;
  const int rel = (int)(blockIdx.x - e.block0);
  const int nt = rel / e.ctiles, ct = rel % e.ctiles;
  const int n0 = nt * PACK_NT, c0 = ct * CT;
  const int run = CT * taps, stride = run + 1;
  const unsigned tmul = e.taps_mul, tshr = e.taps_shr, lgct = e.ct_log2;
  for (int i = threadIdx.x; i < PACK_NT * run; i += 256) {
    const int nl = fast_div(i >> lgct, tmul, tshr), r = i - nl * run;
    const int n = n0 + nl, c = c0 + fast_div(r, tmul, tshr);
    float v = 0.f;
    if (n < Cout && c < CinReal) v = w[(unsigned)((n * CinReal + c0) * taps + r)];
    tile[nl * stride + r] = v;
  }
  __syncthreads();
  if (e.has_f) {
    for (int i = threadIdx.x; i < PACK_NT * run; i += 256) {
      const int cl = i & (CT - 1), q = i >> lgct;
      const int nl = fast_div(q, tmul, tshr), tap = q - nl * taps;
      const int n = n0 + nl, c = c0 + cl;
      if (n < CoutPad && c < Cin)
        pack_store<T, X3>(wf, (long)(unsigned)(n * Kpad + tap * Cin + c), (long)CoutPad * Kpad, tile[nl * stride + cl * taps + tap]);
    }
    if (ct == 0) {
      const int k0 = taps * Cin, tail = Kpad - k0;
      for (int i = threadIdx.x; i < PACK_NT * tail; i += 256) {
        const int n = n0 + i / tail;
        if (n < CoutPad) pack_store<T, X3>(wf, (long)n * Kpad + k0 + i % tail, (long)CoutPad * Kpad, 0.f);
      }
    }
  }
  if (e.has_d) {
    for (int i = threadIdx.x; i < PACK_NT * run; i += 256) {
      const int nl = i & (PACK_NT - 1), q = i / PACK_NT;
      const int cl = fast_div(q, tmul, tshr), slot = q - cl * taps;
      const int n = n0 + nl, c = c0 + cl;
      if (c < CinRows && n < CoutD)
        pack_store<T, X3>(wd, (long)(unsigned)(c * KpadD + slot * CoutD + n), (long)CinRows * KpadD,
                          tile[nl * stride + cl * taps + (taps - 1 - dgrad_tap_slot_to_flipped(slot, taps, e.conv_stride))]);
    }
    if (nt == 0) {
      const int k0 = taps * CoutD, tail = KpadD - k0;
      for (int i = threadIdx.x; i < CT * tail; i += 256) {
        const int c = c0 + i / tail;
        if (c < CinRows) pack_store<T, X3>(wd, (long)c * KpadD + k0 + i % tail, (long)CinRows * KpadD, 0.f);
      }
    }
  }
}

int pack_all_launch(int dtype, const float* params, void* ws, const PackTable& t, int blocks,
                    hipStream_t stream) {
  if (t.n == 0 || blocks == 0) return 0;
  if (dtype == D3F_F32)
    hipLaunchKernelGGL((pack_all_kernel<float, false>), dim3(blocks), dim3(256), 0, stream, params, (char*)ws, t);
  else if (dtype == D3F_F32X3)
    hipLaunchKernelGGL((pack_all_kernel<bf16_t, true>), dim3(blocks), dim3(256), 0, stream, params, (char*)ws, t);
  else
    hipLaunchKernelGGL((pack_all_kernel<bf16_t, false>), dim3(blocks), dim3(256), 0, stream, params, (char*)ws, t);
  D3F_HIP(hipGetLastError());
  return 0;
}

}
```

Before: 2042 images/sec.

## Unroll and specialize BN apply/backward, maxpool backward, SSIM, reductions and weight packing

Templates the BN apply and BN backward-apply kernels on residual, mask and dres modes, hoists per-channel coefficients into registers, and unrolls the grid-stride loops so several loads are in flight. Maxpool backward now handles row pairs per thread with a templated accumulate flag. The SSIM loss uses packed float2 math with batched tile loads. Column reductions, the weight-pack fill and the NCHW-to-NHWC conversion get unrolled or vectorised loads. The aim is more memory-level parallelism and less per-element index and branch overhead, at the cost of more template instantiations and registers. Hoisting c0 out of the loop assumes the grid stride times N is a multiple of C.

Result: faster. 2082 images/sec (median of 6 runs) (+2.0%).

```diff
diff --git a/denoising_diffusion_deep_fake_amd/csrc/batchnorm.hip b/denoising_diffusion_deep_fake_amd/csrc/batchnorm.hip
--- a/denoising_diffusion_deep_fake_amd/csrc/batchnorm.hip
+++ b/denoising_diffusion_deep_fake_amd/csrc/batchnorm.hip
@@ -72,6 +72,29 @@
   s2 = (red[1][0] + red[1][1]) + (red[1][2] + red[1][3]);
 }
 
+__device__ __forceinline__ void column_sum2(const float* __restrict__ col, int rows, long ld, double& s1, double& s2) {
+  int t = threadIdx.x;
+  for (; t + 7 * 256 < rows; t += 8 * 256) {
+    float2 v[8];
+#pragma unroll
+    for (int j = 0; j < 8; ++j) v[j] = *reinterpret_cast<const float2*>(col + (long)(t + j * 256) * ld);
+#pragma unroll
+    for (int j = 0; j < 8; ++j) { s1 += (double)v[j].x; s2 += (double)v[j].y; }
+  }
+  for (; t + 3 * 256 < rows; t += 4 * 256) {
+    float2 v[4];
+#pragma unroll
+    for (int j = 0; j < 4; ++j) v[j] = *reinterpret_cast<const float2*>(col + (long)(t + j * 256) * ld);
+#pragma unroll
+    for (int j = 0; j < 4; ++j) { s1 += (double)v[j].x; s2 += (double)v[j].y; }
+  }
+  for (; t < rows; t += 256) {
+    const float2 v = *reinterpret_cast<const float2*>(col + (long)t * ld);
+    s1 += (double)v.x;
+    s2 += (double)v.y;
+  }
+}
+
 __global__ __launch_bounds__(256) void bn_finalize_kernel(
     const float* __restrict__ stats, int tiles, int C, int Cpad, double count,
     const float* __restrict__ gamma, const float* __restrict__ beta, float eps, float momentum,
@@ -85,11 +108,7 @@
   }
   const int c = blockIdx.x;
   double s1 = 0.0, s2 = 0.0;
-  for (int t = threadIdx.x; t < tiles; t += 256) {
-    const float2 v = *reinterpret_cast<const float2*>(stats + ((long)t * Cpad + c) * 2);
-    s1 += (double)v.x;
-    s2 += (double)v.y;
-  }
+  column_sum2(stats + (long)c * 2, tiles, (long)Cpad * 2, s1, s2);
   block_sum2(s1, s2);
   if (threadIdx.x == 0)
     bn_fwd_coef(s1, s2, count, c, gamma, beta, eps, momentum, true, running_mean, running_var, mean_o, invstd_o, scale_o,
@@ -118,7 +137,7 @@
   return 0;
 }
 
-template <typename T>
+template <typename T, int RES>
 __global__ __launch_bounds__(256) void bn_apply_kernel(
     const T* __restrict__ y, const float* __restrict__ scale, const float* __restrict__ shift,
     const T* __restrict__ res, const T* __restrict__ yr, const float* __restrict__ scale_r,
@@ -128,35 +147,52 @@
     net_shift(y, net_ws); net_shift(scale, net_ws); net_shift(shift, net_ws); net_shift(res, net_ws); net_shift(yr, net_ws);
     net_shift(scale_r, net_ws); net_shift(shift_r, net_ws); net_shift(out, net_ws);
   }
-  constexpr int N = V16<T>::N;
-  for (long i = (long)blockIdx.x * 256 + threadIdx.x; i < nvec; i += (long)gridDim.x * 256) {
-    const int c0 = (int)((i * N) % C);
-    float v[N], sc[N], sf[N];
+  constexpr int N = V16<T>::N, U = N == 4 ? 4 : 2;
+  const int c0 = ((int)threadIdx.x * N) % C;
+  float sc[N], sf[N], scr[N], sfr[N];
+#pragma unroll
+  for (int k = 0; k < N; ++k) {
+    sc[k] = scale[c0 + k];
+    sf[k] = shift[c0 + k];
+    scr[k] = RES == 2 ? scale_r[c0 + k] : 0.f;
+    sfr[k] = RES == 2 ? shift_r[c0 + k] : 0.f;
+  }
+  const T* __restrict__ rsrc = RES == 2 ? yr : res;
+  auto one = [&](float (&v)[N], const float (&r)[N]) {
+#pragma unroll
+    for (int k = 0; k < N; ++k) v[k] = v[k] * sc[k] + sf[k];
+    if constexpr (RES == 1) {
+#pragma unroll
+      for (int k = 0; k < N; ++k) v[k] += r[k];
+    } else if constexpr (RES == 2) {
+#pragma unroll
+      for (int k = 0; k < N; ++k) v[k] += r[k] * scr[k] + sfr[k];
+    }
+    if (relu) {
+#pragma unroll
+      for (int k = 0; k < N; ++k) v[k] = fmaxf(v[k], 0.f);
+    }
+  };
+  const long stride = (long)gridDim.x * 256;
+  long i = (long)blockIdx.x * 256 + threadIdx.x;
+  for (; i + (U - 1) * stride < nvec; i += U * stride) {
+    float v[U][N], r[U][N];
+#pragma unroll
+    for (int u = 0; u < U; ++u) {
+      V16<T>::load(y + (i + u * stride) * N, v[u]);
+      if constexpr (RES != 0) V16<T>::load(rsrc + (i + u * stride) * N, r[u]);
+    }
+#pragma unroll
+    for (int u = 0; u < U; ++u) {
+      one(v[u], r[u]);
+      V16<T>::store(out + (i + u * stride) * N, v[u]);
+    }
+  }
+  for (; i < nvec; i += stride) {
+    float v[N], r[N];
     V16<T>::load(y + i * N, v);
-#pragma unroll
-    for (int k = 0; k < N; k += 4) {
-      const float4 a = *reinterpret_cast<const float4*>(scale + c0 + k);
-      const float4 b = *reinterpret_cast<const float4*>(shift + c0 + k);
-      sc[k] = a.x; sc[k + 1] = a.y; sc[k + 2] = a.z; sc[k + 3] = a.w;
-      sf[k] = b.x; sf[k + 1] = b.y; sf[k + 2] = b.z; sf[k + 3] = b.w;
-    }
-#pragma unroll
-    for (int k = 0; k < N; ++k) v[k] = v[k] * sc[k] + sf[k];
-    if (res != nullptr) {
-      float r[N];
-      V16<T>::load(res + i * N, r);
-#pragma unroll
-      for (int k = 0; k < N; ++k) v[k] += r[k];
-    } else if (yr != nullptr) {
-      float r[N];
-      V16<T>::load(yr + i * N, r);
-#pragma unroll
-      for (int k = 0; k < N; ++k) v[k] += r[k] * scale_r[c0 + k] + shift_r[c0 + k];
-    }
-    if (relu) {
-#pragma unroll
-      for (int k = 0; k < N; ++k) v[k] = fmaxf(v[k], 0.f);
-    }
+    if constexpr (RES != 0) V16<T>::load(rsrc + i * N, r);
+    one(v, r);
     V16<T>::store(out + i * N, v);
   }
 }
@@ -255,20 +291,16 @@
   }
   const int c = blockIdx.x;
   double s1 = 0.0, s2 = 0.0;
-  for (int t = threadIdx.x; t < nblocks; t += 256) {
-    const float2 v = *reinterpret_cast<const float2*>(partial + ((long)t * C + c) * 2);
-    s1 += (double)v.x;
-    s2 += (double)v.y;
-  }
+  column_sum2(partial + (long)c * 2, nblocks, (long)C * 2, s1, s2);
   block_sum2(s1, s2);
   if (threadIdx.x == 0) bn_bwd_coef(s1, s2, count, c, C, gamma, invstd, true, dgamma, dbeta, coef);
 }
 
-template <typename T>
+template <typename T, int MASK, int DRES>
 __global__ __launch_bounds__(256) void bn_bwd_apply_kernel(
     const T* __restrict__ dA, const T* __restrict__ a, const T* __restrict__ y,
     const float* __restrict__ mean, const float* __restrict__ invstd, const float* __restrict__ coef,
-    T* __restrict__ dy, T* __restrict__ dres, int dres_acc, long nvec, int C,
+    T* __restrict__ dy, T* __restrict__ dres, long nvec, int C,
     const float* __restrict__ mask_scale, const float* __restrict__ mask_shift, long net_ws) {
   chain_priority();
   if (blockIdx.z != 0) {
@@ -276,37 +308,72 @@
     net_shift(coef, net_ws); net_shift(dy, net_ws); net_shift(dres, net_ws); net_shift(mask_scale, net_ws);
     net_shift(mask_shift, net_ws);
   }
-  constexpr int N = V16<T>::N;
-  for (long i = (long)blockIdx.x * 256 + threadIdx.x; i < nvec; i += (long)gridDim.x * 256) {
-    const int c0 = (int)((i * N) % C);
-    float g[N], yy[N], o[N];
+  constexpr int N = V16<T>::N, U = N == 4 ? 4 : 2;
+  const int c0 = ((int)threadIdx.x * N) % C;
+  float mu[N], is[N], k0[N], k1[N], k2[N], msc[N], msf[N];
+#pragma unroll
+  for (int k = 0; k < N; ++k) {
+    const int c = c0 + k;
+    mu[k] = mean[c];
+    is[k] = invstd[c];
+    k0[k] = coef[c];
+    k1[k] = coef[C + c];
+    k2[k] = coef[2 * C + c];
+    msc[k] = MASK == 1 ? mask_scale[c] : 0.f;
+    msf[k] = MASK == 1 ? mask_shift[c] : 0.f;
+  }
+  auto one = [&](float (&g)[N], const float (&yy)[N], const float (&aa)[N], float (&o)[N]) {
+    if constexpr (MASK == 1) {
+#pragma unroll
+      for (int k = 0; k < N; ++k) g[k] = (yy[k] * msc[k] + msf[k]) > 0.f ? g[k] : 0.f;
+    } else if constexpr (MASK == 2) {
+#pragma unroll
+      for (int k = 0; k < N; ++k) g[k] = aa[k] > 0.f ? g[k] : 0.f;
+    }
+#pragma unroll
+    for (int k = 0; k < N; ++k) {
+      const float xhat = (yy[k] - mu[k]) * is[k];
+      o[k] = k0[k] * (g[k] - k1[k] - xhat * k2[k]);
+    }
+  };
+  const long stride = (long)gridDim.x * 256;
+  long i = (long)blockIdx.x * 256 + threadIdx.x;
+  for (; i + (U - 1) * stride < nvec; i += U * stride) {
+    float g[U][N], yy[U][N], aa[U][N], d[U][N];
+#pragma unroll
+    for (int u = 0; u < U; ++u) {
+      const long e = (i + u * stride) * N;
+      V16<T>::load(dA + e, g[u]);
+      V16<T>::load(y + e, yy[u]);
+      if constexpr (MASK == 2) V16<T>::load(a + e, aa[u]);
+      if constexpr (DRES == 2) V16<T>::load(dres + e, d[u]);
+    }
+#pragma unroll
+    for (int u = 0; u < U; ++u) {
+      const long e = (i + u * stride) * N;
+      float o[N];
+      one(g[u], yy[u], aa[u], o);
+      V16<T>::store(dy + e, o);
+      if constexpr (DRES == 2) {
+#pragma unroll
+        for (int k = 0; k < N; ++k) g[u][k] += d[u][k];
+      }
+      if constexpr (DRES != 0) V16<T>::store(dres + e, g[u]);
+    }
+  }
+  for (; i < nvec; i += stride) {
+    float g[N], yy[N], aa[N], d[N], o[N];
     V16<T>::load(dA + i * N, g);
     V16<T>::load(y + i * N, yy);
-    if (mask_scale != nullptr) {
-#pragma unroll
-      for (int k = 0; k < N; ++k) g[k] = (yy[k] * mask_scale[c0 + k] + mask_shift[c0 + k]) > 0.f ? g[k] : 0.f;
-    } else if (a != nullptr) {
-      float aa[N];
-      V16<T>::load(a + i * N, aa);
-#pragma unroll
-      for (int k = 0; k < N; ++k) g[k] = aa[k] > 0.f ? g[k] : 0.f;
-    }
-#pragma unroll
-    for (int k = 0; k < N; ++k) {
-      const int c = c0 + k;
-      const float xhat = (yy[k] - mean[c]) * invstd[c];
-      o[k] = coef[c] * (g[k] - coef[C + c] - xhat * coef[2 * C + c]);
-    }
+    if constexpr (MASK == 2) V16<T>::load(a + i * N, aa);
+    if constexpr (DRES == 2) V16<T>::load(dres + i * N, d);
+    one(g, yy, aa, o);
     V16<T>::store(dy + i * N, o);
-    if (dres != nullptr) {
-      if (dres_acc) {
-        float d[N];
-        V16<T>::load(dres + i * N, d);
-#pragma unroll
-        for (int k = 0; k < N; ++k) g[k] += d[k];
-      }
-      V16<T>::store(dres + i * N, g);
-    }
+    if constexpr (DRES == 2) {
+#pragma unroll
+      for (int k = 0; k < N; ++k) g[k] += d[k];
+    }
+    if constexpr (DRES != 0) V16<T>::store(dres + i * N, g);
   }
 }
 
@@ -671,9 +738,14 @@
   const BnResidualOps r = residual_ops(L, b);
   by_dtype(L.dtype, [&](auto* typed) {
     typedef std::remove_pointer_t<decltype(typed)> T;
-    hipLaunchKernelGGL(bn_apply_kernel<T>, dim3(grid_for(nvec), 1, nv.nets), dim3(256), 0, stream, (const T*)b.y,
-                       bn_coef(b.coef, L.C, BN_SCALE), bn_coef(b.coef, L.C, BN_SHIFT), (const T*)r.res, (const T*)r.yr,
-                       r.scale_r, r.shift_r, L.relu ? 1 : 0, (T*)b.a, nvec, L.C, nv.ws);
+    auto go = [&](auto kernel) {
+      hipLaunchKernelGGL(kernel, dim3(grid_for(nvec), 1, nv.nets), dim3(256), 0, stream, (const T*)b.y,
+                         bn_coef(b.coef, L.C, BN_SCALE), bn_coef(b.coef, L.C, BN_SHIFT), (const T*)r.res, (const T*)r.yr,
+                         r.scale_r, r.shift_r, L.relu ? 1 : 0, (T*)b.a, nvec, L.C, nv.ws);
+    };
+    if (r.res != nullptr) go(bn_apply_kernel<T, 1>);
+    else if (r.yr != nullptr) go(bn_apply_kernel<T, 2>);
+    else go(bn_apply_kernel<T, 0>);
   });
   D3F_HIP(hipGetLastError());
   return 0;
@@ -727,9 +799,22 @@
   if (nvec == 0) return 0;
   by_dtype(L.dtype, [&](auto* typed) {
     typedef std::remove_pointer_t<decltype(typed)> T;
-    hipLaunchKernelGGL(bn_bwd_apply_kernel<T>, dim3(grid_for(nvec), 1, nv.nets), dim3(256), 0, stream, (const T*)b.dA,
-                       (const T*)o.a, (const T*)b.y, o.mean, o.invstd, o.k, (T*)b.dy, (T*)b.dres, b.dres_acc, nvec, C,
-                       o.mask_scale, o.mask_shift, nv.ws);
+    auto go = [&](auto kernel) {
+      hipLaunchKernelGGL(kernel, dim3(grid_for(nvec), 1, nv.nets), dim3(256), 0, stream, (const T*)b.dA, (const T*)o.a,
+                         (const T*)b.y, o.mean, o.invstd, o.k, (T*)b.dy, (T*)b.dres, nvec, C, o.mask_scale, o.mask_shift,
+                         nv.ws);
+    };
+    const int mask = o.mask_scale != nullptr ? 1 : (o.a != nullptr ? 2 : 0);
+    const int dres = b.dres == nullptr ? 0 : (b.dres_acc ? 2 : 1);
+    auto by_dres = [&](auto m) {
+      constexpr int M = decltype(m)::value;
+      if (dres == 0) go(bn_bwd_apply_kernel<T, M, 0>);
+      else if (dres == 1) go(bn_bwd_apply_kernel<T, M, 1>);
+      else go(bn_bwd_apply_kernel<T, M, 2>);
+    };
+    if (mask == 0) by_dres(std::integral_constant<int, 0>());
+    else if (mask == 1) by_dres(std::integral_constant<int, 1>());
+    else by_dres(std::integral_constant<int, 2>());
   });
   D3F_HIP(hipGetLastError());
   return 0;
diff --git a/denoising_diffusion_deep_fake_amd/csrc/loss.hip b/denoising_diffusion_deep_fake_amd/csrc/loss.hip
--- a/denoising_diffusion_deep_fake_amd/csrc/loss.hip
+++ b/denoising_diffusion_deep_fake_amd/csrc/loss.hip
@@ -7,10 +7,12 @@
 constexpr int SS_K = 11;
 constexpr int SS_IN = SS_T + SS_K - 1;
 constexpr int SS_LD = SS_IN + 1;
+constexpr int SS_FILL = (SS_IN * SS_IN + 255) / 256;
 
 struct GaussK {
   float g[SS_K];
 };
+typedef float f32x2 __attribute__((ext_vector_type(2)));
 
 static GaussK make_gauss() {
   GaussK k;
@@ -45,47 +47,59 @@
   const float* __restrict__ px = pred + (long)plane * H * W;
   const float* __restrict__ py = target + (long)plane * H * W;
   const int tid = threadIdx.x;
-  for (int e = tid; e < SS_IN * SS_IN; e += 256) {
-    const int r = e / SS_IN, c = e - r * SS_IN;
-    const int iy = oy0 + r, ix = ox0 + c;
-    float a = 0.f, b = 0.f;
-    if (iy < H && ix < W) {
-      a = norm01(px[(long)iy * W + ix], lo, range);
-      b = norm01(py[(long)iy * W + ix], lo, range);
-    }
-    tx[r * SS_LD + c] = a;
-    ty[r * SS_LD + c] = b;
+  {
+    float ra[SS_FILL], rb[SS_FILL];
+#pragma unroll
+    for (int k = 0; k < SS_FILL; ++k) {
+      const int e = tid + k * 256, r = e / SS_IN, c = e - r * SS_IN;
+      const int iy = oy0 + r, ix = ox0 + c;
+      const long off = (e < SS_IN * SS_IN && iy < H && ix < W) ? (long)iy * W + ix : 0;
+      ra[k] = px[off];
+      rb[k] = py[off];
+    }
+#pragma unroll
+    for (int k = 0; k < SS_FILL; ++k) {
+      const int e = tid + k * 256, r = e / SS_IN, c = e - r * SS_IN;
+      const int iy = oy0 + r, ix = ox0 + c;
+      if (e < SS_IN * SS_IN) {
+        const bool in = iy < H && ix < W;
+        tx[r * SS_LD + c] = in ? norm01(ra[k], lo, range) : 0.f;
+        ty[r * SS_LD + c] = in ? norm01(rb[k], lo, range) : 0.f;
+      }
+    }
   }
   __syncthreads();
   constexpr int RB = 8;
   if (tid < SS_IN * (SS_T / RB)) {
     const int c = tid % SS_IN, r0 = (tid / SS_IN) * RB;
-    float a[RB + SS_K - 1], b[RB + SS_K - 1], aa[RB + SS_K - 1], bb[RB + SS_K - 1], ab[RB + SS_K - 1];
+    f32x2 xy[RB + SS_K - 1], sq[RB + SS_K - 1];
+    float ab[RB + SS_K - 1];
 #pragma unroll
     for (int i = 0; i < RB + SS_K - 1; ++i) {
-      a[i] = tx[(r0 + i) * SS_LD + c];
-      b[i] = ty[(r0 + i) * SS_LD + c];
-      aa[i] = a[i] * a[i];
-      bb[i] = b[i] * b[i];
-      ab[i] = a[i] * b[i];
-    }
-#pragma unroll
-    for (int r = 0; r < RB; ++r) {
-      float s0 = 0.f, s1 = 0.f, s2 = 0.f, s3 = 0.f, s4 = 0.f;
+      xy[i] = f32x2{tx[(r0 + i) * SS_LD + c], ty[(r0 + i) * SS_LD + c]};
+      sq[i] = xy[i] * xy[i];
+      ab[i] = xy[i].x * xy[i].y;
+    }
+#pragma unroll
+    for (int r = 0; r < RB; r += 2) {
+      f32x2 s01[2] = {f32x2{0.f, 0.f}, f32x2{0.f, 0.f}}, s23[2] = {f32x2{0.f, 0.f}, f32x2{0.f, 0.f}}, s4 = f32x2{0.f, 0.f};
 #pragma unroll
       for (int i = 0; i < SS_K; ++i) {
-        const float g = gk.g[i];
-        s0 += g * a[r + i];
-        s1 += g * b[r + i];
-        s2 += g * aa[r + i];
-        s3 += g * bb[r + i];
-        s4 += g * ab[r + i];
+        const f32x2 g = f32x2{gk.g[i], gk.g[i]};
+        s01[0] += g * xy[r + i];
+        s23[0] += g * sq[r + i];
+        s01[1] += g * xy[r + 1 + i];
+        s23[1] += g * sq[r + 1 + i];
+        s4 += g * f32x2{ab[r + i], ab[r + 1 + i]};
       }
-      vv[0][(r0 + r) * SS_LD + c] = s0;
-      vv[1][(r0 + r) * SS_LD + c] = s1;
-      vv[2][(r0 + r) * SS_LD + c] = s2;
-      vv[3][(r0 + r) * SS_LD + c] = s3;
-      vv[4][(r0 + r) * SS_LD + c] = s4;
+#pragma unroll
+      for (int e = 0; e < 2; ++e) {
+        vv[0][(r0 + r + e) * SS_LD + c] = s01[e].x;
+        vv[1][(r0 + r + e) * SS_LD + c] = s01[e].y;
+        vv[2][(r0 + r + e) * SS_LD + c] = s23[e].x;
+        vv[3][(r0 + r + e) * SS_LD + c] = s23[e].y;
+        vv[4][(r0 + r + e) * SS_LD + c] = e ? s4.y : s4.x;
+      }
     }
   }
   __syncthreads();
@@ -93,24 +107,39 @@
   float local = 0.f;
   constexpr int CBk = 4;
   const int rr = tid / (SS_T / CBk), cq = (tid % (SS_T / CBk)) * CBk;
-  float win[5][CBk + SS_K - 1];
-#pragma unroll
-  for (int q = 0; q < 5; ++q)
-#pragma unroll
-    for (int j = 0; j < CBk + SS_K - 1; ++j) win[q][j] = vv[q][rr * SS_LD + cq + j];
+  f32x2 w01[CBk + SS_K - 1], w23[CBk + SS_K - 1];
+  float w4[CBk + SS_K - 1];
+#pragma unroll
+  for (int j = 0; j < CBk + SS_K - 1; ++j) {
+    w01[j] = f32x2{vv[0][rr * SS_LD + cq + j], vv[1][rr * SS_LD + cq + j]};
+    w23[j] = f32x2{vv[2][rr * SS_LD + cq + j], vv[3][rr * SS_LD + cq + j]};
+    w4[j] = vv[4][rr * SS_LD + cq + j];
+  }
+  float mm[CBk][5];
+#pragma unroll
+  for (int cc = 0; cc < CBk; cc += 2) {
+    f32x2 s01[2] = {f32x2{0.f, 0.f}, f32x2{0.f, 0.f}}, s23[2] = {f32x2{0.f, 0.f}, f32x2{0.f, 0.f}}, s4 = f32x2{0.f, 0.f};
+#pragma unroll
+    for (int j = 0; j < SS_K; ++j) {
+      const f32x2 g = f32x2{gk.g[j], gk.g[j]};
+      s01[0] += g * w01[cc + j];
+      s23[0] += g * w23[cc + j];
+      s01[1] += g * w01[cc + 1 + j];
+      s23[1] += g * w23[cc + 1 + j];
+      s4 += g * f32x2{w4[cc + j], w4[cc + 1 + j]};
+    }
+#pragma unroll
+    for (int e = 0; e < 2; ++e) {
+      mm[cc + e][0] = s01[e].x; mm[cc + e][1] = s01[e].y; mm[cc + e][2] = s23[e].x; mm[cc + e][3] = s23[e].y;
+      mm[cc + e][4] = e ? s4.y : s4.x;
+    }
+  }
 #pragma unroll
   for (int cc = 0; cc < CBk; ++cc) {
     const int r = rr, c = cq + cc;
     const int oy = oy0 + r, ox = ox0 + c;
     if (oy >= Hv || ox >= Wv) continue;
-    float m[5];
-#pragma unroll
-    for (int q = 0; q < 5; ++q) {
-      float s = 0.f;
-#pragma unroll
-      for (int j = 0; j < SS_K; ++j) s += gk.g[j] * win[q][cc + j];
-      m[q] = s;
-    }
+    const float (&m)[5] = mm[cc];
     const float mux = m[0], muy = m[1];
     const float sxx = m[2] - mux * mux, syy = m[3] - muy * muy, sxy = m[4] - mux * muy;
     const float a1 = 2.f * mux * muy + c1, b1 = mux * mux + muy * muy + c1;
@@ -147,71 +176,103 @@
   const int plane = blockIdx.z;
   const int py0 = blockIdx.y * SS_T, px0 = blockIdx.x * SS_T;
   const int tid = threadIdx.x;
-  for (int e = tid; e < SS_IN * SS_IN; e += 256) {
-    const int r = e / SS_IN, c = e - r * SS_IN;
-    const int oy = py0 - (SS_K - 1) + r, ox = px0 - (SS_K - 1) + c;
-    float a = 0.f, b = 0.f, d = 0.f;
-    if (oy >= 0 && oy < Hv && ox >= 0 && ox < Wv) {
-      const long o = ((long)plane * Hv + oy) * Wv + ox;
-      a = dA[o];
-      b = dB[o];
-      d = dC[o];
-    }
-    t3[0][r * SS_LD + c] = a;
-    t3[1][r * SS_LD + c] = b;
-    t3[2][r * SS_LD + c] = d;
+  constexpr int CBk = 4;
+  const int rr = tid / (SS_T / CBk), cq = (tid % (SS_T / CBk)) * CBk;
+  float pv4[CBk], tv4[CBk];
+  {
+    float ra[SS_FILL], rb[SS_FILL], rd[SS_FILL];
+#pragma unroll
+    for (int k = 0; k < SS_FILL; ++k) {
+      const int e = tid + k * 256, r = e / SS_IN, c = e - r * SS_IN;
+      const int oy = py0 - (SS_K - 1) + r, ox = px0 - (SS_K - 1) + c;
+      const bool in = e < SS_IN * SS_IN && oy >= 0 && oy < Hv && ox >= 0 && ox < Wv;
+      const long o = (long)plane * Hv * Wv + (in ? (long)oy * Wv + ox : 0);
+      ra[k] = dA[o];
+      rb[k] = dB[o];
+      rd[k] = dC[o];
+    }
+#pragma unroll
+    for (int cc = 0; cc < CBk; ++cc) {
+      const int iy = py0 + rr, ix = px0 + cq + cc;
+      const long p = (long)plane * H * W + ((iy < H && ix < W) ? (long)iy * W + ix : 0);
+      pv4[cc] = pred[p];
+      tv4[cc] = target[p];
+    }
+#pragma unroll
+    for (int k = 0; k < SS_FILL; ++k) {
+      const int e = tid + k * 256, r = e / SS_IN, c = e - r * SS_IN;
+      const int oy = py0 - (SS_K - 1) + r, ox = px0 - (SS_K - 1) + c;
+      if (e < SS_IN * SS_IN) {
+        const bool in = oy >= 0 && oy < Hv && ox >= 0 && ox < Wv;
+        t3[0][r * SS_LD + c] = in ? ra[k] : 0.f;
+        t3[1][r * SS_LD + c] = in ? rb[k] : 0.f;
+        t3[2][r * SS_LD + c] = in ? rd[k] : 0.f;
+      }
+    }
   }
   __syncthreads();
   constexpr int RB = 8;
   if (tid < SS_IN * (SS_T / RB)) {
     const int c = tid % SS_IN, r0 = (tid / SS_IN) * RB;
-    float v0[RB + SS_K - 1], v1[RB + SS_K - 1], v2[RB + SS_K - 1];
+    f32x2 v01[RB + SS_K - 1];
+    float v2[RB + SS_K - 1];
 #pragma unroll
     for (int i = 0; i < RB + SS_K - 1; ++i) {
-      v0[i] = t3[0][(r0 + i) * SS_LD + c];
-      v1[i] = t3[1][(r0 + i) * SS_LD + c];
+      v01[i] = f32x2{t3[0][(r0 + i) * SS_LD + c], t3[1][(r0 + i) * SS_LD + c]};
       v2[i] = t3[2][(r0 + i) * SS_LD + c];
     }
 #pragma unroll
-    for (int r = 0; r < RB; ++r) {
-      float s0 = 0.f, s1 = 0.f, s2 = 0.f;
+    for (int r = 0; r < RB; r += 2) {
+      f32x2 s01[2] = {f32x2{0.f, 0.f}, f32x2{0.f, 0.f}}, s2 = f32x2{0.f, 0.f};
 #pragma unroll
       for (int i = 0; i < SS_K; ++i) {
-        const float g = gk.g[SS_K - 1 - i];
-        s0 += g * v0[r + i];
-        s1 += g * v1[r + i];
-        s2 += g * v2[r + i];
+        const f32x2 g = f32x2{gk.g[SS_K - 1 - i], gk.g[SS_K - 1 - i]};
+        s01[0] += g * v01[r + i];
+        s01[1] += g * v01[r + 1 + i];
+        s2 += g * f32x2{v2[r + i], v2[r + 1 + i]};
       }
-      vv[0][(r0 + r) * SS_LD + c] = s0;
-      vv[1][(r0 + r) * SS_LD + c] = s1;
-      vv[2][(r0 + r) * SS_LD + c] = s2;
+#pragma unroll
+      for (int e = 0; e < 2; ++e) {
+        vv[0][(r0 + r + e) * SS_LD + c] = s01[e].x;
+        vv[1][(r0 + r + e) * SS_LD + c] = s01[e].y;
+        vv[2][(r0 + r + e) * SS_LD + c] = e ? s2.y : s2.x;
+      }
     }
   }
   __syncthreads();
   const float inv_range = 1.f / range;
   float local = 0.f;
-  constexpr int CBk = 4;
-  const int rr = tid / (SS_T / CBk), cq = (tid % (SS_T / CBk)) * CBk;
-  float win[3][CBk + SS_K - 1];
-#pragma unroll
-  for (int q = 0; q < 3; ++q)
-#pragma unroll
-    for (int j = 0; j < CBk + SS_K - 1; ++j) win[q][j] = vv[q][rr * SS_LD + cq + j];
+  f32x2 w01[CBk + SS_K - 1];
+  float w2[CBk + SS_K - 1];
+#pragma unroll
+  for (int j = 0; j < CBk + SS_K - 1; ++j) {
+    w01[j] = f32x2{vv[0][rr * SS_LD + cq + j], vv[1][rr * SS_LD + cq + j]};
+    w2[j] = vv[2][rr * SS_LD + cq + j];
+  }
+  float gg[CBk][3];
+#pragma unroll
+  for (int cc = 0; cc < CBk; cc += 2) {
+    f32x2 s01[2] = {f32x2{0.f, 0.f}, f32x2{0.f, 0.f}}, s2 = f32x2{0.f, 0.f};
+#pragma unroll
+    for (int j = 0; j < SS_K; ++j) {
+      const f32x2 g = f32x2{gk.g[SS_K - 1 - j], gk.g[SS_K - 1 - j]};
+      s01[0] += g * w01[cc + j];
+      s01[1] += g * w01[cc + 1 + j];
+      s2 += g * f32x2{w2[cc + j], w2[cc + 1 + j]};
+    }
+#pragma unroll
+    for (int e = 0; e < 2; ++e) {
+      gg[cc + e][0] = s01[e].x; gg[cc + e][1] = s01[e].y; gg[cc + e][2] = e ? s2.y : s2.x;
+    }
+  }
 #pragma unroll
   for (int cc = 0; cc < CBk; ++cc) {
     const int r = rr, c = cq + cc;
     const int iy = py0 + r, ix = px0 + c;
     if (iy >= H || ix >= W) continue;
-    float ga = 0.f, gb = 0.f, gc = 0.f;
-#pragma unroll
-    for (int j = 0; j < SS_K; ++j) {
-      const float g = gk.g[SS_K - 1 - j];
-      ga += g * win[0][cc + j];
-      gb += g * win[1][cc + j];
-      gc += g * win[2][cc + j];
-    }
+    const float ga = gg[cc][0], gb = gg[cc][1], gc = gg[cc][2];
     const long p = (long)plane * H * W + (long)iy * W + ix;
-    const float pv = pred[p], tv = target[p];
+    const float pv = pv4[cc], tv = tv4[cc];
     const float rawx = (pv - lo) / range;
     const float xh = fminf(fmaxf(rawx, 0.f), 1.f);
     const float yh = norm01(tv, lo, range);
@@ -236,9 +297,17 @@
                                                             double n_elems, float* __restrict__ out) {
   chain_priority();
   __shared__ double red[2][256];
-  double a = 0.0, b = 0.0;
-  for (int i = threadIdx.x; i < n_ss; i += 256) a += (double)part_ss[i];
-  for (int i = threadIdx.x; i < n_mse; i += 256) b += (double)part_mse[i];
+  auto strided_sum = [](const float* __restrict__ p, int n) {
+    double s = 0.0;
+    int i = threadIdx.x;
+    for (; i + 3 * 256 < n; i += 4 * 256) {
+      const float v0 = p[i], v1 = p[i + 256], v2 = p[i + 512], v3 = p[i + 768];
+      s += (double)v0; s += (double)v1; s += (double)v2; s += (double)v3;
+    }
+    for (; i < n; i += 256) s += (double)p[i];
+    return s;
+  };
+  const double a = strided_sum(part_ss, n_ss), b = strided_sum(part_mse, n_mse);
   red[0][threadIdx.x] = a;
   red[1][threadIdx.x] = b;
   __syncthreads();
diff --git a/denoising_diffusion_deep_fake_amd/csrc/pointwise.hip b/denoising_diffusion_deep_fake_amd/csrc/pointwise.hip
--- a/denoising_diffusion_deep_fake_amd/csrc/pointwise.hip
+++ b/denoising_diffusion_deep_fake_amd/csrc/pointwise.hip
@@ -1,6 +1,8 @@
 #include "pointwise.h"
 #include "philox.h"
 #include "vec16.h"
+
+#include <type_traits>
 
 namespace d3f {
 
@@ -53,10 +55,11 @@
   }
 }
 
-template <typename T>
+constexpr int MPB_PAIRS = 2;
+template <typename T, bool ACC>
 __global__ __launch_bounds__(256) void maxpool_bwd_kernel(const T* __restrict__ dout,
                                                           const uint8_t* __restrict__ idx,
-                                                          T* __restrict__ din, int accumulate, int B,
+                                                          T* __restrict__ din, int npairs,
                                                           int H, int W, int C, unsigned vc_mul, unsigned vc_shr,
                                                           long net_ws) {
   chain_priority();
@@ -68,48 +71,69 @@
   const int j = (int)blockIdx.x * 256 + (int)threadIdx.x;
   if (j >= W * VC) return;
   const int ix = fast_div(j, vc_mul, vc_shr), cv = j - ix * VC;
-  const int row = (int)blockIdx.y;
-  const int iy = row % H, b = row / H;
-  const int noy = (iy & 1) ? 2 : 1, nox = (ix & 1) ? 2 : 1;
-  const int oy0 = (iy + 1) >> 1, kh0 = (iy & 1) ? 0 : 1;
-  const int ox0 = (ix + 1) >> 1, kw0 = (ix & 1) ? 0 : 1;
-  float g[N];
-#pragma unroll
-  for (int k = 0; k < N; ++k) g[k] = 0.f;
-#pragma unroll
-  for (int a = 0; a < 2; ++a) {
-    const int oy = oy0 - a, kh = a ? 2 : kh0;
-    if (a >= noy || oy >= Ho) continue;
-#pragma unroll
-    for (int c = 0; c < 2; ++c) {
-      const int ox = ox0 - c, kw = c ? 2 : kw0;
-      if (c < nox && ox < Wo) {
-        const long o = (((long)b * Ho + oy) * Wo + ox) * C + cv * N;
-        float d[N];
-        V16<T>::load(dout + o, d);
-        const unsigned tap = (unsigned)(kh * 3 + kw);
-        uint32_t w[N / 4];
+  const int ox0 = (ix + 1) >> 1;
+  const bool okc[2] = {ox0 < Wo, (ix & 1) != 0};
+  const int oxc[2] = {ox0 < Wo ? ox0 : Wo - 1, ox0 > 0 ? ox0 - 1 : 0};
+  const unsigned kwc[2] = {(ix & 1) ? 0u : 1u, 2u};
+  float d[MPB_PAIRS][2][2][N], old[MPB_PAIRS][2][N];
+  uint32_t w[MPB_PAIRS][2][2][N / 4];
+  bool next[MPB_PAIRS];
+#pragma unroll
+  for (int u = 0; u < MPB_PAIRS; ++u) {
+    int p = (int)blockIdx.y * MPB_PAIRS + u;
+    if (p >= npairs) p = npairs - 1;
+    next[u] = p % Ho + 1 < Ho;
+#pragma unroll
+    for (int a = 0; a < 2; ++a) {
+      const long prow = a && next[u] ? p + 1 : p;
+#pragma unroll
+      for (int c = 0; c < 2; ++c) {
+        const long o = (prow * Wo + oxc[c]) * C + cv * N;
+        V16<T>::load(dout + o, d[u][a][c]);
         if constexpr (N == 4) {
-          w[0] = *reinterpret_cast<const uint32_t*>(idx + o);
+          w[u][a][c][0] = *reinterpret_cast<const uint32_t*>(idx + o);
         } else {
           const uint2 t = *reinterpret_cast<const uint2*>(idx + o);
-          w[0] = t.x;
-          w[1] = t.y;
+          w[u][a][c][0] = t.x;
+          w[u][a][c][1] = t.y;
         }
-#pragma unroll
-        for (int k = 0; k < N; ++k)
-          if (((w[k >> 2] >> (8 * (k & 3))) & 0xffu) == tap) g[k] += d[k];
-      }
-    }
-  }
-  T* dst = din + ((long)row * W * VC + j) * N;
-  if (accumulate) {
-    float old[N];
-    V16<T>::load(dst, old);
-#pragma unroll
-    for (int k = 0; k < N; ++k) g[k] += old[k];
-  }
-  V16<T>::store(dst, g);
+      }
+    }
+    if constexpr (ACC) {
+#pragma unroll
+      for (int e = 0; e < 2; ++e) V16<T>::load(din + ((2L * p + e) * W * VC + j) * N, old[u][e]);
+    }
+  }
+#pragma unroll
+  for (int u = 0; u < MPB_PAIRS; ++u) {
+    const int p = (int)blockIdx.y * MPB_PAIRS + u;
+    if (p >= npairs) break;
+    float g[2][N];
+#pragma unroll
+    for (int k = 0; k < N; ++k) g[0][k] = g[1][k] = 0.f;
+    auto add = [&](float (&gr)[N], int a, unsigned kh, bool row_ok) {
+#pragma unroll
+      for (int c = 0; c < 2; ++c) {
+        const unsigned tap = kh * 3 + kwc[c];
+#pragma unroll
+        for (int k = 0; k < N; ++k) {
+          const bool hit = row_ok && okc[c] && ((w[u][a][c][k >> 2] >> (8 * (k & 3))) & 0xffu) == tap;
+          gr[k] = hit ? gr[k] + d[u][a][c][k] : gr[k];
+        }
+      }
+    };
+    add(g[0], 0, 1, true);
+    add(g[1], 1, 0, next[u]);
+    add(g[1], 0, 2, true);
+#pragma unroll
+    for (int e = 0; e < 2; ++e) {
+      if constexpr (ACC) {
+#pragma unroll
+        for (int k = 0; k < N; ++k) g[e][k] += old[u][e][k];
+      }
+      V16<T>::store(din + ((2L * p + e) * W * VC + j) * N, g[e]);
+    }
+  }
 }
 
 int maxpool3x3s2_fwd_launch(int dtype, const void* in, void* out, uint8_t* idx, int B, int H, int W,
@@ -141,13 +165,20 @@
   unsigned vc_mul, vc_shr;
   fast_div_setup((unsigned)vc, &vc_mul, &vc_shr);
   D3F_CHECK((long)B * H <= 65535, "maxpool backward: %d rows exceed the grid", B * H);
-  const dim3 grid((unsigned)cdiv((long)W * vc, 256), (unsigned)(B * H), (unsigned)nv.nets);
-  if (dtype == D3F_F32)
-    hipLaunchKernelGGL(maxpool_bwd_kernel<float>, grid, dim3(256), 0, stream,
-                       (const float*)dout, idx, (float*)din, accumulate, B, H, W, C, vc_mul, vc_shr, nv.ws);
-  else
-    hipLaunchKernelGGL(maxpool_bwd_kernel<bf16_t>, grid, dim3(256), 0, stream,
-                       (const bf16_t*)dout, idx, (bf16_t*)din, accumulate, B, H, W, C, vc_mul, vc_shr, nv.ws);
+  const int npairs = B * (H / 2);
+  const dim3 grid((unsigned)cdiv((long)W * vc, 256), (unsigned)cdiv(npairs, MPB_PAIRS), (unsigned)nv.nets);
+  auto go = [&](auto kernel, auto* typed) {
+    typedef std::remove_pointer_t<decltype(typed)> T;
+    hipLaunchKernelGGL(kernel, grid, dim3(256), 0, stream, (const T*)dout, idx, (T*)din, npairs, H, W, C, vc_mul, vc_shr,
+                       nv.ws);
+  };
+  if (dtype == D3F_F32) {
+    if (accumulate) go(maxpool_bwd_kernel<float, true>, (float*)nullptr);
+    else go(maxpool_bwd_kernel<float, false>, (float*)nullptr);
+  } else {
+    if (accumulate) go(maxpool_bwd_kernel<bf16_t, true>, (bf16_t*)nullptr);
+    else go(maxpool_bwd_kernel<bf16_t, false>, (bf16_t*)nullptr);
+  }
   D3F_HIP(hipGetLastError());
   return 0;
 }
@@ -210,6 +241,17 @@
     net_shift(in, net_in); net_shift(out, net_ws);
   }
   const long total = (long)B * HW;
+  constexpr int N = V16<T>::N;
+  if (Cpad == N && C <= N && (reinterpret_cast<uintptr_t>(out) & 15) == 0) {
+    for (long i = (long)blockIdx.x * 256 + threadIdx.x; i < total; i += (long)gridDim.x * 256) {
+      const long b = i / HW, pix = i - b * HW;
+      alignas(16) T px[N];
+#pragma unroll
+      for (int c = 0; c < N; ++c) px[c] = from_f32<T>(c < C ? in[(b * C + c) * HW + pix] : 0.f);
+      *reinterpret_cast<uint4*>(out + i * N) = *reinterpret_cast<const uint4*>(px);
+    }
+    return;
+  }
   for (long i = (long)blockIdx.x * 256 + threadIdx.x; i < total; i += (long)gridDim.x * 256) {
     const long b = i / HW, pix = i - b * HW;
     for (int c = 0; c < Cpad; ++c) {
@@ -580,12 +622,23 @@
   const int n0 = nt * PACK_NT, c0 = ct * CT;
   const int run = CT * taps, stride = run + 1;
   const unsigned tmul = e.taps_mul, tshr = e.taps_shr, lgct = e.ct_log2;
-  for (int i = threadIdx.x; i < PACK_NT * run; i += 256) {
-    const int nl = fast_div(i >> lgct, tmul, tshr), r = i - nl * run;
-    const int n = n0 + nl, c = c0 + fast_div(r, tmul, tshr);
-    float v = 0.f;
-    if (n < Cout && c < CinReal) v = w[(unsigned)((n * CinReal + c0) * taps + r)];
-    tile[nl * stride + r] = v;
+  constexpr int LU = 8;
+  for (int i0 = threadIdx.x; i0 < PACK_NT * run; i0 += 256 * LU) {
+    float v[LU];
+    int dst[LU];
+#pragma unroll
+    for (int u = 0; u < LU; ++u) {
+      const int i = i0 + u * 256;
+      const int nl = fast_div(i >> lgct, tmul, tshr), r = i - nl * run;
+      const int n = n0 + nl, c = c0 + fast_div(r, tmul, tshr);
+      dst[u] = i < PACK_NT * run ? nl * stride + r : -1;
+      const bool real = dst[u] >= 0 && n < Cout && c < CinReal;
+      const float x = w[real ? (unsigned)((n * CinReal + c0) * taps + r) : 0u];
+      v[u] = real ? x : 0.f;
+    }
+#pragma unroll
+    for (int u = 0; u < LU; ++u)
+      if (dst[u] >= 0) tile[dst[u]] = v[u];
   }
   __syncthreads();
   if (e.has_f) {
```
